# fuxiao0719/PanopticNeRF

Hardware: AMD Instinct MI355X
Metric: Msamples/sec (coarse+fine), KITTI-360 1408x376 (higher is better)
Workload: dtype bf16

## Files before the change

include/pnr.h:

```cpp
#ifndef PNR_H
#define PNR_H
#include <stdint.h>

#ifdef __cplusplus
extern "C" {
#endif

#define PNR_OK 0
#define PNR_EINVAL (-1)
#define PNR_EHIP (-2)
#define PNR_ENODEV (-3)

#define PNR_PREC_BF16 0
#define PNR_PREC_FP32 1

int pnr_version(void);
const char* pnr_last_error(void);
int pnr_device_check(int dev, char* buf_host, int buflen);

int pnr_stratified(const float* rays, int64_t n_rays, int n_samples, int lindisp,
                   const float* t_rand, float* z_out, void* stream);

int pnr_points(const float* rays, const float* z, int64_t n_rays, int n_samples, float* pts_out,
               void* stream);

int pnr_embed(const float* x, int64_t n, int L, float* out, void* stream);

typedef struct pnr_mlp_desc {
    int32_t D, W, skip;
    int32_t xyz_L, dir_L;
    int32_t n_sem, n_inst, head_W;
    int32_t precision;
    int32_t plan;
    int32_t head_tap;
    int32_t head_depth;
    int32_t schedule;
    int32_t clk_probe[2];
    int32_t flags;
} pnr_mlp_desc;

#define PNR_MLP_SOFTMAX 1
#define PNR_MLP_WG_CAP(n) (((n) & 0x1FF) << 16)
#define PNR_MLP_TRACE 0x7A00

typedef struct pnr_mlp_params_host {
    const float* const* pts_w; const float* const* pts_b;
    const float* alpha_w; const float* alpha_b;
    const float* feature_w; const float* feature_b;
    const float* views_w; const float* views_b;
    const float* rgb_w; const float* rgb_b;
    const float* sem0_w; const float* sem0_b; const float* sem1_w; const float* sem1_b;
    const float* inst0_w; const float* inst0_b; const float* inst1_w; const float* inst1_b;
} pnr_mlp_params_host;

int64_t pnr_mlp_packed_bytes(const pnr_mlp_desc* desc);
int pnr_mlp_pack(const pnr_mlp_desc* desc, const pnr_mlp_params_host* params, void* packed_host);

int64_t pnr_mlp_pack_workspace_bytes(const pnr_mlp_desc* desc, int backward);
int pnr_mlp_pack_device(const pnr_mlp_desc* desc, const pnr_mlp_params_host* params_dev, int backward,
                        void* workspace, void* packed, void* stream);
int pnr_mlp_repack_device(const pnr_mlp_desc* desc, const pnr_mlp_params_host* params_dev, int backward,
                          void* workspace, void* packed, void* stream);

int pnr_mlp_forward(const pnr_mlp_desc* desc, const void* packed, const float* rays, const float* z,
                    int64_t n_rays, int n_samples, float* raw, int64_t raw_stride_s,
                    int64_t raw_stride_c, void* stream);

int pnr_mlp_fused_plan(const pnr_mlp_desc* desc);
int64_t pnr_mlp_forward_composite_workspace_bytes(const pnr_mlp_desc* desc, int64_t n_rays, int n_samples, int want_weights);
int pnr_mlp_forward_composite(const pnr_mlp_desc* desc, const void* packed, const float* rays, const float* z,
                              int64_t n_rays, int n_samples, const int32_t* label_sem, const int32_t* label_inst,
                              int white_bkgd, float* rgb, float* depth, float* acc, float* weights, float* sem,
                              float* inst, float* fix_sem, float* fix_inst, void* workspace, void* stream);

int pnr_mlp_forward_tiles(const pnr_mlp_desc* desc, const void* packed, const float* rays, const float* z, int64_t n_rays,
                          int n_samples, void* workspace, void* stream);
int pnr_composite_combine(const pnr_mlp_desc* desc, const void* workspace, const float* z, int64_t n_rays, int n_samples,
                          const int32_t* label_sem, const int32_t* label_inst, int white_bkgd, float* rgb, float* depth,
                          float* acc, float* weights, float* sem, float* inst, float* fix_sem, float* fix_inst, void* stream);

int pnr_mlp_query(const pnr_mlp_desc* desc, const void* packed, const float* points, int64_t n_points,
                  float* sigma, int32_t* sem_label, int32_t* inst_label, int32_t* panoptic, const int32_t* is_thing,
                  float* sem_logits, float* inst_logits, int64_t logit_stride, void* stream);
int pnr_mlp_query_supported(const pnr_mlp_desc* desc);

int pnr_mlp_train_layout(const pnr_mlp_desc* desc, int64_t n_samples, int64_t* acts_off_host ,
                         int64_t* dys_off_host );
int pnr_mlp_forward_train(const pnr_mlp_desc* desc, const void* packed, const float* rays, const float* z,
                          int64_t n_rays, int n_samples, float* raw, int64_t raw_stride_s,
                          int64_t raw_stride_c, void* acts, void* stream);
int64_t pnr_mlp_bwd_packed_bytes(const pnr_mlp_desc* desc);
int pnr_mlp_pack_bwd(const pnr_mlp_desc* desc, const pnr_mlp_params_host* params, void* packed_host);
int pnr_mlp_backward(const pnr_mlp_desc* desc, const void* packed_bwd, const float* d_raw, const void* acts,
                     void* dys, int64_t n_rays, int n_samples, void* stream);

int64_t pnr_mlp_wgrad_workspace_bytes(const pnr_mlp_desc* desc, int64_t n_samples);
int pnr_mlp_wgrad(const pnr_mlp_desc* desc, const void* acts, const void* dys, int64_t n_samples,
                  const pnr_mlp_params_host* grads_dev, void* workspace, void* stream);

int64_t pnr_mlp_fp32_acts_floats(const pnr_mlp_desc* desc, int64_t n_samples);
int64_t pnr_mlp_backward_fp32_workspace_bytes(const pnr_mlp_desc* desc, int64_t n_samples);
int pnr_mlp_forward_train_fp32(const pnr_mlp_desc* desc, const pnr_mlp_params_host* params_dev, const float* rays,
                               const float* z, int64_t n_rays, int n_samples, float* raw, int64_t raw_stride_s,
                               int64_t raw_stride_c, float* acts, void* stream);
int pnr_mlp_backward_fp32(const pnr_mlp_desc* desc, const pnr_mlp_params_host* params_dev, const float* d_raw,
                          int64_t d_raw_stride_c, const float* acts, int64_t n_rays, int n_samples,
                          const pnr_mlp_params_host* grads_dev, void* workspace, void* stream);

int pnr_composite(const float* raw, int64_t raw_stride_s, int64_t raw_stride_c, const float* z,
                  const float* rays, const float* noise, const int32_t* label_sem,
                  const int32_t* label_inst, int64_t n_rays, int n_samples, int n_sem, int n_inst,
                  int sem_mode, int white_bkgd, float* rgb, float* depth, float* acc, float* weights,
                  float* sem, float* inst, float* fix_sem, float* fix_inst, void* stream);

int pnr_composite_backward(const float* raw, int64_t raw_stride_c, const float* z, const float* rays,
                           const float* noise, int64_t n_rays, int n_samples, int n_sem, int n_inst,
                           const float* g_rgb, const float* g_depth, const float* g_acc, const float* g_sem,
                           const float* g_inst, const float* g_weights, float* d_raw, void* stream);

int pnr_composite_backward2(const float* raw, int64_t raw_stride_c, const float* z, const float* rays,
                            const float* noise, int64_t n_rays, int n_samples, int n_sem, int n_inst,
                            const float* g_rgb, const float* g_depth, const float* g_acc, const float* g_sem,
                            const float* g_inst, const float* g_weights, const int32_t* label_sem,
                            const int32_t* label_inst, const float* g_fix_sem, const float* g_fix_inst,
                            const float* ce_sem, const float* ce_inst, float* d_raw, void* stream);
// ... 244 lines not shown
```

panopticnerf_amd/_lib.py:

```python
import ctypes
import os

_HERE = os.path.dirname(os.path.abspath(__file__))
LIB_PATH = os.environ.get("PNR_LIB_PATH") or os.path.join(_HERE, "libpnr.so")

c_f = ctypes.c_void_p
c_i64 = ctypes.c_int64
c_int = ctypes.c_int

PREC_BF16, PREC_FP32 = 0, 1
MLP_SOFTMAX, MLP_TRACE = 1, 0x7A00
CAMERA_PINHOLE, CAMERA_FISHEYE, CAMERA_EQUIRECT = 0, 1, 3
TAG_PIXEL, TAG_FRAME = 16, 17
SAMPLE_POOLED, SAMPLE_FRAME = 0, 1
NORMAL_OK, NORMAL_NO_DEPTH, NORMAL_NO_NEIGHBOUR, NORMAL_DEGENERATE, NORMAL_GRAZING = 0, 1, 2, 3, 4
DEPTH_MAX_RADIUS = 8
NN_MAX_TABLE, CLOUD_MAX_TAU, SAMPLE_MAX_PER_FACE = 1 << 28, 8, 65535


class LossCfg(ctypes.Structure):
    _fields_ = [("w_rgb", ctypes.c_float), ("w_depth", ctypes.c_float), ("w_sem", ctypes.c_float),
                ("w_fix_sem", ctypes.c_float), ("w_inst", ctypes.c_float), ("w_fix_inst", ctypes.c_float),
                ("depth_l2", ctypes.c_int32), ("fix_eps", ctypes.c_float), ("maps_are_prob", ctypes.c_int32)]


class MlpDesc(ctypes.Structure):
    _fields_ = [("D", ctypes.c_int32), ("W", ctypes.c_int32), ("skip", ctypes.c_int32),
                ("xyz_L", ctypes.c_int32), ("dir_L", ctypes.c_int32),
                ("n_sem", ctypes.c_int32), ("n_inst", ctypes.c_int32), ("head_W", ctypes.c_int32),
                ("precision", ctypes.c_int32), ("plan", ctypes.c_int32), ("head_tap", ctypes.c_int32),
                ("head_depth", ctypes.c_int32), ("schedule", ctypes.c_int32), ("clk_probe", ctypes.c_int32 * 2), ("flags", ctypes.c_int32)]


class RngDesc(ctypes.Structure):
    _fields_ = [("call", ctypes.c_void_p), ("ray_base", ctypes.c_int64), ("tag", ctypes.c_int32), ("scale", ctypes.c_float)]


class Frame(ctypes.Structure):
    _fields_ = [("model", ctypes.c_int32), ("width", ctypes.c_int32), ("height", ctypes.c_int32), ("cam", ctypes.c_float * 7),
                ("c2w", ctypes.c_float * 12), ("near_", ctypes.c_float), ("far_", ctypes.c_float), ("n_valid", ctypes.c_int64),
                ("valid_pix", ctypes.c_uint64), ("rgb", ctypes.c_uint64), ("depth", ctypes.c_uint64), ("sem", ctypes.c_uint64),
                ("inst", ctypes.c_uint64)]


_fp = ctypes.POINTER(ctypes.c_float)
_fpp = ctypes.POINTER(_fp)


class MlpParamsHost(ctypes.Structure):
    _fields_ = [("pts_w", _fpp), ("pts_b", _fpp),
                ("alpha_w", _fp), ("alpha_b", _fp), ("feature_w", _fp), ("feature_b", _fp),
                ("views_w", _fp), ("views_b", _fp), ("rgb_w", _fp), ("rgb_b", _fp),
                ("sem0_w", _fp), ("sem0_b", _fp), ("sem1_w", _fp), ("sem1_b", _fp),
                ("inst0_w", _fp), ("inst0_b", _fp), ("inst1_w", _fp), ("inst1_b", _fp)]


SIGNATURES = {
    "pnr_version": (c_int, []),
    "pnr_last_error": (ctypes.c_char_p, []),
    "pnr_device_check": (c_int, [c_int, ctypes.c_char_p, c_int]),
    "pnr_stratified": (c_int, [c_f, c_i64, c_int, c_int, c_f, c_f, c_f]),
    "pnr_points": (c_int, [c_f, c_f, c_i64, c_int, c_f, c_f]),
    "pnr_embed": (c_int, [c_f, c_i64, c_int, c_f, c_f]),
    "pnr_mlp_packed_bytes": (c_i64, [ctypes.POINTER(MlpDesc)]),
    "pnr_mlp_pack": (c_int, [ctypes.POINTER(MlpDesc), ctypes.POINTER(MlpParamsHost), ctypes.c_void_p]),
    "pnr_mlp_pack_workspace_bytes": (c_i64, [ctypes.POINTER(MlpDesc), c_int]),
    "pnr_mlp_pack_device": (c_int, [ctypes.POINTER(MlpDesc), ctypes.POINTER(MlpParamsHost), c_int, c_f, c_f, c_f]),
    "pnr_mlp_repack_device": (c_int, [ctypes.POINTER(MlpDesc), ctypes.POINTER(MlpParamsHost), c_int, c_f, c_f, c_f]),
    "pnr_mlp_forward": (c_int, [ctypes.POINTER(MlpDesc), c_f, c_f, c_f, c_i64, c_int, c_f, c_i64, c_i64, c_f]),
    "pnr_mlp_train_layout": (c_int, [ctypes.POINTER(MlpDesc), c_i64, ctypes.POINTER(c_i64), ctypes.POINTER(c_i64)]),
    "pnr_mlp_forward_train": (c_int, [ctypes.POINTER(MlpDesc), c_f, c_f, c_f, c_i64, c_int, c_f, c_i64, c_i64, c_f, c_f]),
    "pnr_mlp_bwd_packed_bytes": (c_i64, [ctypes.POINTER(MlpDesc)]),
    "pnr_mlp_pack_bwd": (c_int, [ctypes.POINTER(MlpDesc), ctypes.POINTER(MlpParamsHost), ctypes.c_void_p]),
    "pnr_mlp_backward": (c_int, [ctypes.POINTER(MlpDesc), c_f, c_f, c_f, c_f, c_i64, c_int, c_f]),
    "pnr_mlp_wgrad_workspace_bytes": (c_i64, [ctypes.POINTER(MlpDesc), c_i64]),
    "pnr_mlp_wgrad": (c_int, [ctypes.POINTER(MlpDesc), c_f, c_f, c_i64, ctypes.POINTER(MlpParamsHost), c_f, c_f]),
    "pnr_mlp_fp32_acts_floats": (c_i64, [ctypes.POINTER(MlpDesc), c_i64]),
    "pnr_mlp_backward_fp32_workspace_bytes": (c_i64, [ctypes.POINTER(MlpDesc), c_i64]),
    "pnr_mlp_forward_train_fp32": (c_int, [ctypes.POINTER(MlpDesc), ctypes.POINTER(MlpParamsHost), c_f, c_f, c_i64, c_int, c_f, c_i64,
                                           c_i64, c_f, c_f]),
    "pnr_mlp_backward_fp32": (c_int, [ctypes.POINTER(MlpDesc), ctypes.POINTER(MlpParamsHost), c_f, c_i64, c_f, c_i64, c_int,
                                      ctypes.POINTER(MlpParamsHost), c_f, c_f]),
    "pnr_mlp_fused_plan": (c_int, [ctypes.POINTER(MlpDesc)]),
    "pnr_mlp_forward_composite_workspace_bytes": (c_i64, [ctypes.POINTER(MlpDesc), c_i64, c_int, c_int]),
    "pnr_mlp_forward_composite": (c_int, [ctypes.POINTER(MlpDesc), c_f, c_f, c_f, c_i64, c_int, c_f, c_f, c_int,
                                          c_f, c_f, c_f, c_f, c_f, c_f, c_f, c_f, c_f, c_f]),
    "pnr_composite": (c_int, [c_f, c_i64, c_i64, c_f, c_f, c_f, c_f, c_f, c_i64, c_int, c_int, c_int, c_int,
                              c_int, c_f, c_f, c_f, c_f, c_f, c_f, c_f, c_f, c_f]),
    "pnr_composite_backward": (c_int, [c_f, c_i64, c_f, c_f, c_f, c_i64, c_int, c_int, c_int,
                                       c_f, c_f, c_f, c_f, c_f, c_f, c_f, c_f]),
    "pnr_composite_backward2": (c_int, [c_f, c_i64, c_f, c_f, c_f, c_i64, c_int, c_int, c_int,
                                        c_f, c_f, c_f, c_f, c_f, c_f, c_f, c_f, c_f, c_f, c_f, c_f, c_f, c_f]),
    "pnr_composite_backward3": (c_int, [c_f, c_i64, c_f, c_f, c_f, c_i64, c_int, c_int, c_int, c_int,
                                        c_f, c_f, c_f, c_f, c_f, c_f, c_f, c_f, c_f, c_f, c_f, c_f, c_f, c_f]),
# ... 105 lines not shown
```

panopticnerf_amd/csrc/asm/gen_mlp_tt.py:

```python
#!/usr/bin/env python3
import struct
import sys
from contextlib import contextmanager

V_T2 = 15
NSLOT, SLOT = 4, 33 * 1024
P = 4
D, SKIP = 8, 4

V_TID, V_LANE16, V_FRAG, V_BIAS, V_T0, V_DMA, V_LB4, V_TRACE = 0, 1, 2, 6, 10, 11, 14, 15
V_T1 = 1
V_RING, V_ACC = 16, 32
V_EX, V_ED = 160, 192
V_G = 208
V_ZZ, V_ZN, V_DN, V_LW = 240, 242, 244, 246
V_IN = 224
V_TMP = 208
V_PTMP = 248
V_AUXA = V_PTMP + 6
V_LWA = V_IN + 2
A0, A1 = 0, 128
S_IMG, S_RAYS, S_Z, S_S, S_N, S_MAGIC, S_SHIFT, S_NGRP, S_NWG, S_REC, S_RECF, S_PS, S_NSEM, S_NINST, S_CLK = 4, 6, 8, 10, 11, 12, 13, 14, 15, 16, 18, 20, 22, 23, 24
S_WAVE, S_W4K, S_GRP, S_PIECE, S_T0, S_T1 = 26, 27, 28, 30, 34, 35
S_VALID, S_LAST = 36, 40
S_NVALID, S_NLAST = 44, 48
S_LO32, S_N0, S_HI0 = 52, 54, 56
S_SAVE, S_REC_T = 58, 60
S_MSK = 64
S_REC_I = 70
S_AUX = 82
S_VMSK = 76
S_LWW, S_LWR = 74, 75
LW_BASE = NSLOT * SLOT
S_CLK0 = 96
S_K = 100
S_Q = 19
S_GRP2 = 29


def f32(x):
    return struct.unpack("<I", struct.pack("<f", x))[0]


def vr(lo, n):
    return "v[%d:%d]" % (lo, lo + n - 1) if n > 1 else "v%d" % lo


def ar(lo, n):
    return "a[%d:%d]" % (lo, lo + n - 1) if n > 1 else "a%d" % lo


def sr(lo, n=2):
    return "s[%d:%d]" % (lo, lo + n - 1) if n > 1 else "s%d" % lo


class Loc:
    def __init__(self, kind, base):
        self.kind, self.base = kind, base

    def reg(self, i, n=1):
        return (ar if self.kind == "a" else vr)(self.base + i, n)


class Sim:
    def __init__(self, name, cap):
        self.name, self.cap, self.q, self.n = name, cap, [], 0

    def push(self, certain=True):
        self.n += 1
        self.q.append((self.n, certain))
        return self.n

    def wait_count(self, tag):
        if tag is None or not any(t == tag for t, _ in self.q):
            return None
        idx = [t for t, _ in self.q].index(tag)
        n = sum(1 for _, c in self.q[idx + 1:] if c)
        n = min(n, self.cap)
        self.q = self.q[idx + 1:]
        return n

    def drain(self):
        self.q = []

    def state(self):
        return [c for _, c in self.q]


class Gen:
    def __init__(self, nbs, nbi, name, trace=False, abl=0, depth=2, softmax=False, tap=0):
        self.depth = depth
        self.tap = tap
        self.softmax = softmax
        self.nbs, self.nbi, self.name, self.trace, self.abl = nbs, nbi, name, trace, abl
        self.nstamp = 0
        self.o = []
        self.nlabel = 0
        self.lgkm = Sim("lgkm", 15)
        self.vm = Sim("vm", 63)
        self.side, self.side_lo, self.outbox, self.capture = [], [], [], None
        self.ring_tags = [None] * P
        self.piece_tag = {}
        self.pending_pack = None
        self.g2_acc = self.park_acc = None
        self.m0 = None
        self.logit_units = []
        self.acc_free = list(range(8))
        self.lwr_acc = self.lwr_tag = None
        self.aux_tags = {}
        self.build_plan()
        self.build_units()
        self.stream = []
        for u in self.units:
            u["frag0"] = len(self.stream)
            self.stream += [(sl, of) for sl, of, _, _ in self.unit_frags(u)]

    def build_plan(self):
        L = []

        def add(name, nblk, segs, fbc, mode):
            nks = sum(n for _, n in segs)
            if fbc * nks + 1 > 33:
                fbc = 1
            L.append(dict(name=name, nblk=nblk, segs=segs, nks=nks, fbc=fbc, mode=mode))
        for i in range(D):
            if i == 0:
                add("L0", 8, [("ex", 4)], 8, "relu")
            elif i - 1 == SKIP:
                add("L%d" % i, 8, [("ex", 4), ("h", 16)], 2, "relu")
            else:
                add("L%d" % i, 8, [("h", 16)], 2, "relu")
        add("feature", 8, [("h", 16)], 2, "linear")
        add("views", 4, [("F", 16), ("ed", 2)], 2, "relu")
        add("rgbs", 1, [("g", 8), ("hh", 16)], 1, "rgbs")
        if self.depth == 1:
            if self.nbs:
                add("sem1", self.nbs, [("tap", 16)], self.nbs, "logits")
            if self.nbi:
                add("inst1", 1, [("tap", 16)], 1, "logits")
        else:
            if self.nbs:
                add("sem0", 4, [("tap", 16)], 2, "relu")
            if self.nbi:
                add("inst0", 4, [("tap", 16)], 2, "relu")
            if self.nbs:
                add("sem1", self.nbs, [("shs", 8)], self.nbs, "logits")
            if self.nbi:
                add("inst1", 1, [("shi", 8)], 1, "logits")
        self.layers = L
        self.chunks = []
        off = 0
        for li, l in enumerate(L):
            for fb in range(0, l["nblk"], l["fbc"]):
                nfrag = l["fbc"] * l["nks"] + 1
                self.chunks.append(dict(layer=li, fb=fb, nfb=l["fbc"], off=off, nfrag=nfrag))
                off += nfrag
        self.total_frags = off
        while len(self.chunks) % NSLOT:
            self.chunks.append(dict(layer=None, fb=0, nfb=0, off=0, nfrag=1, dummy=True))
        self.NC = len(self.chunks)
        assert self.NC % NSLOT == 0, self.NC
        assert max(c["nfrag"] for c in self.chunks) <= 33

    class Holder:
        def __init__(self, v=None):
            self.v = v

    def e(self, s):
        if self.capture is not None:
            self.capture.append("\t" + s)
        else:
            self.o.append("\t" + s)

# ... 229 lines not shown
        e("v_fma_f32 v%d, -v%d, v%d, v%d" % (a, a, q_, b))
        e("v_div_fmas_f32 v%d, v%d, v%d, v%d" % (a, a, r, q_))
        e("v_div_fixup_f32 v%d, v%d, v%d, v%d" % (res, a, den, num))

    def sqrt(self, res, x, t):
        y, ym, tt = t[:3]
        e = self.e
        self.lit(S_K, 0x0f800000)
        e("v_mul_f32 v%d, 0x4f800000, v%d" % (tt, x))
        e("v_cmp_gt_f32 vcc, s%d, v%d" % (S_K, x))
        e("v_cndmask_b32 v%d, v%d, v%d, vcc" % (x, x, tt))
        e("v_sqrt_f32 v%d, v%d" % (y, x))
        e("s_nop 0")
        e("v_add_u32 v%d, -1, v%d" % (ym, y))
        e("v_fma_f32 v%d, -v%d, v%d, v%d" % (tt, ym, y, x))
        e("v_cmp_ge_f32 s[%d:%d], 0, v%d" % (S_T0, S_T0 + 1, tt))
        e("v_cndmask_b32 v%d, v%d, v%d, s[%d:%d]" % (ym, y, ym, S_T0, S_T0 + 1))
        e("v_add_u32 v%d, 1, v%d" % (tt, y))
        e("v_fma_f32 v%d, -v%d, v%d, v%d" % (y, tt, y, x))
        e("v_cmp_lt_f32 s[%d:%d], 0, v%d" % (S_T0, S_T0 + 1, y))
        e("v_cndmask_b32 v%d, v%d, v%d, s[%d:%d]" % (ym, ym, tt, S_T0, S_T0 + 1))
        e("v_mul_f32 v%d, 0x37800000, v%d" % (tt, ym))
        e("v_cndmask_b32 v%d, v%d, v%d, vcc" % (ym, ym, tt))
        e("v_mov_b32 v%d, 0x260" % tt)
        e("v_cmp_class_f32 vcc, v%d, v%d" % (x, tt))
        e("v_cndmask_b32 v%d, v%d, v%d, vcc" % (res, ym, x))

    def sincos(self, s_out, c_out, x, t):
        kf, r, r2, a, b, ki = t[:6]
        e = self.e
        C = dict(twoopi=f32(0.636619772367581343), c1=f32(1.57079637050628662109375), c2=f32(-4.371139000186241e-08),
                 s3=f32(-1.9515295891e-4), s2=f32(8.3321608736e-3), s1=f32(-1.6666654611e-1),
                 c4=f32(2.443315711809948e-5), c3=f32(-1.388731625493765e-3), c2b=f32(4.166664568298827e-2))
        assert C["twoopi"] == 0x3f22f983 and C["c1"] == 0x3fc90fdb and C["c2"] == 0xb33bbd2e and C["s3"] == 0xb94ca1f9
        assert C["s2"] == 0x3c08839e and C["s1"] == 0xbe2aaaa3 and C["c4"] == 0x37ccf5ce and C["c3"] == 0xbab6061a and C["c2b"] == 0x3d2aaaa5
        e("v_mul_f32 v%d, 0x%x, v%d" % (kf, C["twoopi"], x))
        e("v_rndne_f32 v%d, v%d" % (kf, kf))
        e("v_mov_b32 v%d, v%d" % (r, x))
        e("v_fmac_f32 v%d, 0x%x, v%d" % (r, C["c1"] ^ 0x80000000, kf))
        e("v_fmac_f32 v%d, 0x%x, v%d" % (r, C["c2"] ^ 0x80000000, kf))
        e("v_cvt_i32_f32 v%d, v%d" % (ki, kf))
        e("v_mul_f32 v%d, v%d, v%d" % (r2, r, r))
        e("v_mov_b32 v%d, 0x%x" % (a, C["s2"]))
        e("v_fmac_f32 v%d, 0x%x, v%d" % (a, C["s3"], r2))
        e("v_fmaak_f32 v%d, v%d, v%d, 0x%x" % (a, r2, a, C["s1"]))
        e("v_mul_f32 v%d, v%d, v%d" % (b, r, r2))
        e("v_fma_f32 v%d, v%d, v%d, v%d" % (a, b, a, r))
        e("v_mov_b32 v%d, 0x%x" % (b, C["c3"]))
        e("v_fmac_f32 v%d, 0x%x, v%d" % (b, C["c4"], r2))
        e("v_fmaak_f32 v%d, v%d, v%d, 0x%x" % (b, r2, b, C["c2b"]))
        e("v_fma_f32 v%d, v%d, v%d, -0.5" % (b, r2, b))
        e("v_fma_f32 v%d, v%d, v%d, 1.0" % (b, r2, b))
        e("v_and_b32 v%d, 1, v%d" % (r, ki))
        e("v_cmp_eq_u32 vcc, 0, v%d" % r)
        e("v_cndmask_b32 v%d, v%d, v%d, vcc" % (r2, b, a))
        e("v_cndmask_b32 v%d, v%d, v%d, vcc" % (kf, a, b))
        e("v_and_b32 v%d, 2, v%d" % (a, ki))
        e("v_lshlrev_b32 v%d, 30, v%d" % (a, a))
        e("v_xor_b32 v%d, v%d, v%d" % (s_out, r2, a))
        e("v_add_u32 v%d, 1, v%d" % (a, ki))
        e("v_and_b32 v%d, 2, v%d" % (a, a))
        e("v_lshlrev_b32 v%d, 30, v%d" % (a, a))
        e("v_xor_b32 v%d, v%d, v%d" % (c_out, kf, a))

    def band_pack(self, dst3, s, c):
        e = self.e
        e("v_cvt_pk_bf16_f32 v%d, v%d, v%d" % (dst3, s[0], s[1]))
        e("v_cvt_pk_bf16_f32 v%d, v%d, v%d" % (dst3 + 1, s[2], c[0]))
        e("v_cvt_pk_bf16_f32 v%d, v%d, v%d" % (dst3 + 2, c[1], c[2]))

    def band_next(self, s, c, t):
        e = self.e
        for a in range(3):
            e("v_add_f32 v%d, v%d, v%d" % (t, s[a], s[a]))
            e("v_mul_f32 v%d, v%d, v%d" % (t, t, c[a]))
            e("v_mul_f32 v%d, -2.0, v%d" % (c[a], s[a]))
            e("v_fma_f32 v%d, v%d, v%d, 1.0" % (c[a], c[a], s[a]))
            e("v_mov_b32 v%d, v%d" % (s[a], t))

    def fetch_tile(self, t, grp_sreg):
        e = self.e
        vi = V_IN + 8 * t
        s_, sl, ray, a64 = V_PTMP, V_PTMP + 1, V_PTMP + 2, V_PTMP + 4
        e("s_lshl_b32 s%d, s%d, 3" % (S_T0, grp_sreg))
        e("s_lshl_b32 s%d, s%d, 1" % (S_T1, S_WAVE))
        e("s_add_u32 s%d, s%d, s%d" % (S_T0, S_T0, S_T1))
        e("s_add_u32 s%d, s%d, %d" % (S_T0, S_T0, t))
        e("s_lshl_b32 s%d, s%d, 5" % (S_T0, S_T0))
        e("v_and_b32 v%d, 31, v%d" % (s_, V_TID))
        e("v_or_b32 v%d, s%d, v%d" % (s_, S_T0, s_))
        e("v_cmp_gt_i32 s[%d:%d], s%d, v%d" % (S_NVALID + 2 * t, S_NVALID + 2 * t + 1, S_S, s_))
        e("s_add_i32 s%d, s%d, -1" % (S_T1, S_S))
        e("v_min_i32 v%d, s%d, v%d" % (sl, S_T1, s_))
        e("v_mul_hi_u32 v%d, v%d, s%d" % (ray, sl, S_MAGIC))
        e("v_mul_lo_u32 v%d, v%d, s%d" % (a64, sl, S_MAGIC))
        e("v_mov_b32 v%d, v%d" % (a64 + 1, ray))
        e("v_lshrrev_b64 v[%d:%d], s%d, v[%d:%d]" % (a64, a64 + 1, S_SHIFT, a64, a64 + 1))
        e("v_mov_b32 v%d, v%d" % (ray, a64))
        e("v_mul_lo_u32 v%d, v%d, s%d" % (a64, ray, S_N))
        e("v_sub_u32 v%d, v%d, v%d" % (a64, sl, a64))
        e("v_add_u32 v%d, 1, v%d" % (a64, a64))
        e("v_cmp_eq_u32 s[%d:%d], s%d, v%d" % (S_NLAST + 2 * t, S_NLAST + 2 * t + 1, S_N, a64))
        e("v_lshlrev_b32 v%d, 7, v%d" % (V_AUXA + t, ray))
        e("v_and_b32 v%d, 32, v%d" % (a64, V_TID))
        e("v_lshl_add_u32 v%d, v%d, 1, v%d" % (V_AUXA + t, a64, V_AUXA + t))
        e("v_lshlrev_b32 v%d, 5, v%d" % (a64, ray))
        self.vm_op("global_load_dwordx4 %s, v%d, s[%d:%d]" % (vr(vi, 4), a64, S_RAYS, S_RAYS + 1))
        self.vm_op("global_load_dwordx2 %s, v%d, s[%d:%d] offset:16" % (vr(vi + 4, 2), a64, S_RAYS, S_RAYS + 1))
        e("v_lshlrev_b32 v%d, 2, v%d" % (a64, sl))
        self.vm_op("global_load_dword v%d, v%d, s[%d:%d]" % (vi + 6, a64, S_Z, S_Z + 1))
        e("v_add_u32 v%d, 1, v%d" % (a64 + 1, sl))
        e("v_cmp_gt_i32 vcc, s%d, v%d" % (S_S, a64 + 1))
        e("v_cndmask_b32 v%d, v%d, v%d, vcc" % (a64 + 1, sl, a64 + 1))
        e("v_lshlrev_b32 v%d, 2, v%d" % (a64 + 1, a64 + 1))
        return self.vm_op("global_load_dword v%d, v%d, s[%d:%d]" % (vi + 7, a64 + 1, S_Z, S_Z + 1))

    def encode_tile(self, t, part):
        vi = V_IN + 8 * t
        T = list(range(V_TMP, V_TMP + 16))
        s = T[0:3]
        c = T[3:6]
        q = T[6:9]
        w = T[9:15]
        tt = T[15]
        e = self.e
        ex, ed = V_EX + 16 * t, V_ED + 8 * t
        out = []

        def hi_select(dst, v_hi1, v_hi0):
            e("v_cndmask_b32 v%d, v%d, v%d, s[%d:%d]" % (dst, v_hi1, v_hi0, S_HI0, S_HI0 + 1))

        def points():
            for a in range(3):
                e("v_mul_f32 v%d, v%d, v%d" % (q[a], vi + 3 + a, vi + 6))
                e("v_add_f32 v%d, v%d, v%d" % (q[a], vi + a, q[a]))
        if part == "x":
            out.append((6, points))

        def aux_x():
            self.aux_tags[t] = self.vm_op("global_load_dword v%d, v%d, s[%d:%d] offset:32" % (vi + 0, V_AUXA + t, S_AUX, S_AUX + 1))
            e("v_mov_b32 v%d, v%d" % (vi + 3, V_AUXA + t))
        if part == "x":
            out.append((2, aux_x))

        def xyz_reg():
            hi_select(w[0], q[2], q[0])
            e("v_mov_b32 v%d, 0" % w[1])
            hi_select(w[1], w[1], q[1])
            e("v_cvt_pk_bf16_f32 v%d, v%d, v%d" % (ex, w[0], w[1]))
            e("v_mov_b32 v%d, 0x42000000" % tt)
            e("v_mov_b32 v%d, 1.0" % w[1])
            hi_select(tt, tt, w[1])
            for a in range(3):
                e("v_mul_f32 v%d, v%d, v%d" % (q[a], q[a], tt))
        if part == "x":
            out.append((12, xyz_reg))
            for a in range(3):
                out.append((30, (lambda a=a: self.sincos(s[a], c[a], q[a], w))))
            for fp in range(5):
                out.append((3, (lambda fp=fp: self.band_pack(ex + 1 + 3 * fp, s, c))))
                if fp < 4:
                    out.append((15, (lambda: self.band_next(s, c, tt))))

        if part == "x":
            out.append((1, (lambda: self.wait_vm(self.aux_tags[t]))))
            return out

        def d_load():
            self.vm_op("global_load_dwordx4 %s, v%d, s[%d:%d]" % (vr(ed, 4), vi + 3, S_AUX, S_AUX + 1))
            self.aux_tags[2 + t] = self.vm_op("global_load_dwordx4 %s, v%d, s[%d:%d] offset:16" % (vr(ed + 4, 4), vi + 3, S_AUX, S_AUX + 1))
        out.append((2, d_load))
        out.append((1, (lambda: self.wait_vm(self.aux_tags[2 + t]))))
        return out

    def rgbs_epilogue(self, t, acc):
        e = self.e
        T = list(range(V_PTMP, V_PTMP + 8))
        d, x, y, n, al, f = T[0], T[1], T[2], T[3], T[4], T[5]
        VAL, LAST = S_VALID + 2 * t, S_LAST + 2 * t

        def alpha():
            e("v_sub_f32 v%d, v%d, v%d" % (d, V_ZN + t, V_ZZ + t))
            e("v_mov_b32 v%d, 0x501502f9" % x)
            e("v_cndmask_b32 v%d, v%d, v%d, s[%d:%d]" % (d, d, x, LAST, LAST + 1))
            e("v_mul_f32 v%d, v%d, -v%d" % (d, d, V_DN + t))
            e("v_max_f32 v%d, v%d, v%d" % (x, acc + 3, acc + 3))
            e("v_max_f32 v%d, 0, v%d" % (x, x))
            e("v_mul_f32 v%d, v%d, v%d" % (x, d, x))
            self.lit(S_K, 0x3fb8aa3b)
            e("v_mul_f32 v%d, 0x3fb8aa3b, v%d" % (y, x))
            e("v_fma_f32 v%d, v%d, s%d, -v%d" % (d, x, S_K, y))
            e("v_rndne_f32 v%d, v%d" % (n, y))
            e("v_fmac_f32 v%d, 0x32a5705f, v%d" % (d, x))
            e("v_sub_f32 v%d, v%d, v%d" % (y, y, n))
            e("v_add_f32 v%d, v%d, v%d" % (y, y, d))
            e("v_exp_f32 v%d, v%d" % (y, y))
            e("v_cvt_i32_f32 v%d, v%d" % (n, n))
            e("s_nop 0")
            e("v_ldexp_f32 v%d, v%d, v%d" % (y, y, n))
            self.lit(S_K, 0xc2ce8ed0)
            e("v_cmp_ngt_f32 s[%d:%d], s%d, v%d" % (S_T0, S_T0 + 1, S_K, x))
            e("v_cndmask_b32 v%d, 0, v%d, s[%d:%d]" % (y, y, S_T0, S_T0 + 1))
            self.lit(S_K, 0x42b17218)
            e("v_cmp_nlt_f32 s[%d:%d], s%d, v%d" % (S_T0, S_T0 + 1, S_K, x))
            e("v_mov_b32 v%d, 0x7f800000" % n)
            e("v_cndmask_b32 v%d, v%d, v%d, s[%d:%d]" % (y, n, y, S_T0, S_T0 + 1))
            e("v_sub_f32 v%d, 1.0, v%d" % (al, y))
            e("v_cndmask_b32 v%d, 0, v%d, s[%d:%d]" % (al, al, VAL, VAL + 1))
            e("v_sub_f32 v%d, 1.0, v%d" % (f, al))
            e("v_add_f32 v%d, 0x2edbe6ff, v%d" % (f, f))
            e("v_mov_b32 v%d, 1.0" % n)
            e("v_cndmask_b32 v%d, v%d, v%d, s[%d:%d]" % (f, n, f, VAL, VAL + 1))
        self.q(36, alpha)

        def scan():
            for ctrl in ("row_shr:1", "row_shr:2", "row_shr:4", "row_shr:8"):
                e("v_mov_b32 v%d, 1.0" % n)
                e("s_nop 1")
                e("v_mov_b32_dpp v%d, v%d %s row_mask:0xf bank_mask:0xf" % (n, f, ctrl))
                e("v_mul_f32 v%d, v%d, v%d" % (f, f, n))
            e("v_mov_b32 v%d, 1.0" % n)
            e("s_nop 1")
            e("v_mov_b32_dpp v%d, v%d row_bcast:15 row_mask:0xa bank_mask:0xf" % (n, f))
            e("v_mul_f32 v%d, v%d, v%d" % (f, f, n))
            e("v_mov_b32 v%d, 1.0" % n)
            e("s_nop 1")
            e("v_readlane_b32 s%d, v%d, 31" % (S_Q, f))
            e("v_mov_b32_dpp v%d, v%d wave_shr:1 row_mask:0xf bank_mask:0xf" % (n, f))
            e("v_cndmask_b32 v%d, v%d, 1.0, s[%d:%d]" % (n, n, S_N0, S_N0 + 1))
            e("v_mul_f32 v%d, v%d, v%d" % (V_LW + t, al, n))
            if self.nbs:
                with self.atomic():
                    e("v_add_u32 v%d, s%d, v%d" % (n, S_LWW, V_LB4))
                    e("s_mov_b64 exec, s[%d:%d]" % (S_HI0, S_HI0 + 1))
                    self.lds_read("ds_write_b32 v%d, v%d offset:%d" % (n, V_LW + t, 128 * t))
                    e("s_mov_b64 exec, -1")
        self.q(26 + (4 if self.nbs else 0), scan)

        def stores():
          with self.atomic():
            e("s_lshl_b32 s%d, s%d, 3" % (S_T0, S_GRP))
            e("s_lshl_b32 s%d, s%d, 1" % (S_SAVE, S_WAVE))
            e("s_add_u32 s%d, s%d, s%d" % (S_T0, S_T0, S_SAVE))
            e("s_add_u32 s%d, s%d, %d" % (S_T0, S_T0, t))
            e("s_mul_i32 s%d, s%d, s%d" % (S_SAVE, S_T0, S_RECF))
            e("s_mul_hi_i32 s%d, s%d, s%d" % (S_SAVE + 1, S_T0, S_RECF))
            e("s_lshl_b64 s[%d:%d], s[%d:%d], 2" % (S_SAVE, S_SAVE + 1, S_SAVE, S_SAVE + 1))
            e("s_add_u32 s%d, s%d, s%d" % (S_REC_T + 2 * t, S_REC, S_SAVE))
            e("s_addc_u32 s%d, s%d, s%d" % (S_REC_T + 2 * t + 1, S_REC + 1, S_SAVE + 1))
            e("s_lshl_b32 s%d, s%d, 2" % (S_SAVE, S_NSEM))
            e("s_add_u32 s%d, s%d, s%d" % (S_REC_I + 2 * t, S_REC_T + 2 * t, S_SAVE))
            e("s_addc_u32 s%d, s%d, 0" % (S_REC_I + 2 * t + 1, S_REC_T + 2 * t + 1))
            e("s_lshl_b32 s%d, s%d, 5" % (S_T0, S_T0))
            e("v_and_b32 v%d, 31, v%d" % (d, V_TID))
            e("v_or_b32 v%d, s%d, v%d" % (d, S_T0, d))
            e("v_lshlrev_b32 v%d, 4, v%d" % (d, d))
            e("v_mov_b32 v%d, v%d" % (T[4], V_LW + t))
            e("v_mov_b32 v%d, v%d" % (T[5], acc + 0))
            e("v_mov_b32 v%d, v%d" % (T[6], acc + 1))
            e("v_mov_b32 v%d, v%d" % (T[7], acc + 2))
            e("s_and_b64 s[%d:%d], s[%d:%d], s[%d:%d]" % (S_SAVE, S_SAVE + 1, VAL, VAL + 1, S_HI0, S_HI0 + 1))
            e("s_mov_b64 exec, s[%d:%d]" % (S_SAVE, S_SAVE + 1))
            self.vm_op("global_store_dwordx4 v%d, %s, s[%d:%d]" % (d, vr(T[4], 4), S_PS, S_PS + 1))
            e("s_mov_b64 exec, 1")
            e("v_mov_b32 v%d, s%d" % (x, S_Q))
            e("v_mov_b32 v%d, 0" % d)
            self.vm_op("global_store_dword v%d, v%d, s[%d:%d]" % (d, x, S_REC_T + 2 * t, S_REC_T + 2 * t + 1))
            e("s_mov_b64 exec, -1")
        self.q(28, stores)

    def acc_reg(self, i):
        return V_ACC + 16 * i

    def acc_take(self, n):
        assert len(self.acc_free) >= n, ("accumulators exhausted", self.acc_free)
        got, self.acc_free = self.acc_free[:n], self.acc_free[n:]
        return got

    def acc_release(self, ids):
        self.acc_free = sorted(set(self.acc_free) | set(ids))

    def arm_plan(self, u):
        c = self.chunks[u["chunk"]]
        l = self.layers[u["layer"]]
        slot = u["chunk"] % NSLOT
        bias_off = c["nfb"] * l["nks"] * 1024
        u["accs"], u["arm_tags"] = {}, []
        plans = []
        for bi, blk in enumerate(u["blocks"]):
            b_in_chunk = blk - c["fb"]
            for t in range(2):
                key = (bi, t)
                ops = []

                def take(key=key):
                    while not self.acc_free and self.side_busy():
                        self.drain_side(8)
                    u["accs"][key] = self.acc_take(1)[0]
                if t == 1:
                    plans.append([take])
                    continue
                if l["mode"] == "logits":
                    def first(key=key, slot=slot, take=take):
                        take()
                        self.e("v_add_u32 v%d, 0x%x, v%d" % (self.acc_reg(u["accs"][key]), slot * SLOT, V_LB4))
                    ops.append(first)
                    for r in list(range(1, 16)) + [0]:
                        ops.append(lambda key=key, r=r, off=bias_off + b_in_chunk * 128: u["arm_tags"].append(
                            self.lds_read("ds_read_b32 v%d, v%d offset:%d" % (self.acc_reg(u["accs"][key]) + r, self.acc_reg(u["accs"][key]), off))))
                else:
                    for m in range(4):
                        def rd(key=key, m=m, off=bias_off + b_in_chunk * 128 + m * 32, take=take):
                            if m == 0:
                                take()
                            a = self.acc_reg(u["accs"][key])
                            u["arm_tags"].append(self.lds_read("ds_read_b128 %s, v%d offset:%d" % (vr(a + 4 * m, 4), V_BIAS + slot, off)))
                        ops.append(rd)
                plans.append(ops)
        return plans

    def pack_ops(self, u):
        l = self.layers[u["layer"]]
        if not self.trace:
            return self.pack_ops_pipelined(u)
        out = []
        for bi, blk in enumerate(u["blocks"]):
            for t in range(2):
                a = self.acc_reg(u["accs"][(bi, t)])
                dst = self.out_block(l, blk, t)
                for p in range(8):
                    def fn(a=a, p=p, dst=dst, relu=(l["mode"] == "relu"), k=len(out)):
                        tmp = V_T0 if (k & 1) else V_T1
                        if dst.kind == "v" and relu:
                            self.e("v_cvt_pk_bf16_f32 v%d, v%d, v%d" % (tmp, a + 2 * p, a + 2 * p + 1))
                            self.e("v_pk_max_i16 v%d, v%d, 0" % (dst.base + p, tmp))
                        elif dst.kind == "v":
                            self.e("v_cvt_pk_bf16_f32 v%d, v%d, v%d" % (dst.base + p, a + 2 * p, a + 2 * p + 1))
                        else:
                            self.e("v_cvt_pk_bf16_f32 v%d, v%d, v%d" % (tmp, a + 2 * p, a + 2 * p + 1))
                            if relu:
                                self.e("v_pk_max_i16 v%d, v%d, 0" % (tmp, tmp))
                            self.e("v_accvgpr_write_b32 a%d, v%d" % (dst.base + p, tmp))
                    out.append(((dst.kind, dst.base + p), fn, u["accs"][(bi, t)]))
        return out

    def pack_ops_pipelined(self, u):
        l = self.layers[u["layer"]]
        relu = l["mode"] == "relu"
        pairs = []
        for bi, blk in enumerate(u["blocks"]):
            for t in range(2):
                a = self.acc_reg(u["accs"][(bi, t)])
# ... 97 lines not shown
                    dls.append(None)
                k += 1
        for kk in range(k, len(plans)):
            for op in plans[kk]:
                musts.append(op)
                dls.append(None)
        lwr_from = None
        if nxt is None and (self.logit_units or l["mode"] == "logits"):
            lwr_from = len(musts)
            for op in self.lwr_ops():
                musts.append(op)
                dls.append(None)
        n = len(musts)
        pos = []
        late = not packs and n > 0 and nxt is not None
        for j in range(n):
            spread = 1 + (j * max(1, nm - 6)) // max(1, n) if not late else (2 * nm) // 3 + (j * max(1, nm // 3 - 5)) // max(1, n)
            pos.append(spread if dls[j] is None else min(spread, max(0, dls[j] - 2)))
        if lwr_from is not None:
            nl = n - lwr_from
            for j in range(lwr_from, n):
                pos[j] = max(pos[j], min(nm - 2, nm // 2 + ((j - lwr_from) * max(1, nm // 2 - 3)) // nl))
        for j in range(n - 2, -1, -1):
            pos[j] = min(pos[j], pos[j + 1])
        must_at = {}
        for j, g in enumerate(pos):
            must_at.setdefault(g, []).append(j)
        piece_at = {}
        cu = [k for k, x in enumerate(U) if x["chunk"] == u["chunk"]]
        c3 = (u["chunk"] + 3) % self.NC
        npieces = self.pieces_of(c3)
        k_in = cu.index(ui)
        mine = [j for j in range(npieces) if (j * len(cu)) // npieces == k_in]
        cost = [3 * sum(1 for j in must_at.get(g, []) if j < n and dls[j] is not None or (j < n and musts[j] in pack_fns)) +
                sum(1 for j in must_at.get(g, [])) for g in range(nm)]
        for idx, j in enumerate(mine):
            span = max(len(mine) + 1, nm - 3)
            lo = 1 + (idx * span) // max(1, len(mine))
            hi = max(lo + 1, 1 + ((idx + 1) * span) // max(1, len(mine)))
            g = min(range(lo, min(hi, nm - 1)), key=lambda x: (cost[x], x))
            cost[g] += 2
            piece_at.setdefault(g, []).append(j)
        first_wait_done = False
        for i in range(nm):
            f, t = i // 2, i % 2
            slot, off, ks, bi = frags[f]
            gi = u["frag0"] + f
            if t == 0:
                if not first_wait_done:
                    for tg in u["arm_tags"][-1:]:
                        self.wait_lgkm(tg)
                    first_wait_done = True
                self.wait_lgkm(self.ring_tags[gi % P])
            tile = self.tile_at(ks, t)
            a = self.acc_reg(u["accs"][(bi, tile)])
            c_in = self.acc_reg(u["accs"][(bi, 0)]) if ks == 0 else a
            bloc = self.b_operand(u, ks, tile)
            ring = vr(V_RING + 4 * (gi % P), 4)
            if swap:
                e("v_mfma_f32_32x32x16_bf16 %s, %s, %s, %s" % (vr(a, 16), bloc.reg(0, 4), ring, vr(c_in, 16)))
            else:
                e("v_mfma_f32_32x32x16_bf16 %s, %s, %s, %s" % (vr(a, 16), ring, bloc.reg(0, 4), vr(c_in, 16)))
            if t == 1:
                gn = gi + P - 1
                if gn < len(self.stream):
                    sl, of = self.stream[gn]
                    self.ring_tags[gn % P] = self.lds_read("ds_read_b128 %s, v%d offset:%d" % (vr(V_RING + 4 * (gn % P), 4), V_FRAG + sl, of))
            for j in must_at.get(i, []):
                musts[j]()
            for j in ([] if self.abl & 1 else piece_at.get(i, [])):
                if j == 0:
                    self.chunk_base(c3)
                tg = self.piece(c3, j)
                self.piece_tag[c3] = tg
            self.drain_side(1 if l["name"].startswith("L") or l["name"] in ("feature", "views") else 3 if late else 2)
        for g in sorted(must_at):
            assert g < nm, (g, nm)
        if l["mode"] in ("relu", "linear"):
            self.pending_pack = dict(ops=self.pack_ops(u), accs=list(u["accs"].values()))
        elif l["mode"] == "rgbs":
            for t in range(2):
                self.rgbs_epilogue(t, self.acc_reg(u["accs"][(0, t)]))
            ids = list(u["accs"].values())
            self.q(0, lambda: self.defer(lambda: self.acc_release(ids)))
            self.queue_inputs_late()
            self.acc_release([self.g2_acc])
            self.g2_acc = None
            if not self.nbs:
                self.unpark()
        else:
            self.logit_units.append(u)
        if u["last_of_chunk"]:
            c2 = (u["chunk"] + 2) % self.NC
            if not self.abl & 2:
                self.wait_vm(self.piece_tag.get(c2))
                e("s_barrier")
            d = u["chunk"] + 1
            while d < self.NC and self.chunks[d].get("dummy"):
                e("; ==== dummy chunk %d (slot %d)" % (d, d % NSLOT))
                c3 = (d + 3) % self.NC
                for j in ([] if self.abl & 1 else range(self.pieces_of(c3))):
                    if j == 0:
                        self.chunk_base(c3)
                    self.piece_tag[c3] = self.piece(c3, j)
                    self.drain_side(2)
                if not self.abl & 2:
                    self.wait_vm(self.piece_tag.get((d + 2) % self.NC))
                    e("s_barrier")
                d += 1

    def tail_softmax(self, blocks, lwr_reg, tag_lwr):
        e = self.e
        M = (V_TMP, V_RING)
        TMP = [V_IN + 10, V_IN + 11, V_IN + 12, V_IN + 13]
        ninf = V_PTMP + 6
        heads = []
        for inst in (False, True):
            hb = [(u, bi, blk) for (u, bi, blk, i2) in blocks if i2 == inst]
            if hb:
                heads.append((inst, hb))
        for t in (0, 1):
            self.wait_lgkm(tag_lwr[t])
        e("v_mov_b32 v%d, 0xff800000" % ninf)

        def xor16(op):
            regs = [M[t] + r for t in (0, 1) for r in range(16)]
            for g in range(0, 32, 4):
                for i in range(4):
                    e("v_mov_b32 v%d, v%d" % (TMP[i], regs[g + i]))
                for i in range(4):
                    e("v_permlane16_swap_b32 v%d, v%d" % (regs[g + i], TMP[i]))
                for i in range(4):
                    e("%s v%d, v%d, v%d" % (op, regs[g + i], regs[g + i], TMP[i]))
        for inst, hb in heads:
            accs = [[self.acc_reg(u["accs"][(bi, t)]) for (u, bi, blk) in hb] for t in (0, 1)]
            NB = len(hb)
            vm = S_VMSK + 2 * (1 if inst else 0)
            for t in (0, 1):
                for r in range(16):
                    e("v_cndmask_b32 v%d, v%d, v%d, s[%d:%d]" % (accs[t][NB - 1] + r, ninf, accs[t][NB - 1] + r, vm, vm + 1))
            first_src = None
            if NB > 1:
                for t in (0, 1):
                    for r in range(16):
                        e("v_max_f32 v%d, v%d, v%d" % (M[t] + r, accs[t][0] + r, accs[t][1] + r))
                        for b in range(2, NB):
                            e("v_max_f32 v%d, v%d, v%d" % (M[t] + r, M[t] + r, accs[t][b] + r))
            else:
                first_src = [accs[t][0] for t in (0, 1)]
            for k, ctrl in enumerate(("quad_perm:[1,0,3,2]", "quad_perm:[2,3,0,1]", "row_half_mirror", "row_mirror")):
                for t in (0, 1):
                    for r in range(16):
                        src = (first_src[t] + r) if (k == 0 and first_src) else (M[t] + r)
                        e("v_max_f32_dpp v%d, v%d, v%d %s row_mask:0xf bank_mask:0xf bound_ctrl:1" % (M[t] + r, src, src, ctrl))
            xor16("v_max_f32")
            for t in (0, 1):
                for r in range(16):
                    e("v_mul_f32 v%d, 0xbfb8aa3b, v%d" % (M[t] + r, M[t] + r))
            for t in (0, 1):
                for r in range(16):
                    for b in range(NB):
                        e("v_fmamk_f32 v%d, v%d, 0x3fb8aa3b, v%d" % (accs[t][b] + r, accs[t][b] + r, M[t] + r))
                        e("v_exp_f32 v%d, v%d" % (accs[t][b] + r, accs[t][b] + r))
            first_src = None
            if NB > 1:
                for t in (0, 1):
                    for r in range(16):
# ... 15 lines not shown
                for r in range(16):
                    e("v_mul_f32 v%d, v%d, v%d" % (M[t] + r, lwr_reg(t, r), M[t] + r))
            for r in range(16):
                for t in (0, 1):
                    for (u, bi, blk) in hb:
                        kk = [i for i, (u2, bi2, blk2, i2) in enumerate(blocks) if u2 is u and bi2 == bi][0]
                        a = self.acc_reg(u["accs"][(bi, t)])
                        dst = self.sm_sums[t][kk]
                        if r == 0:
                            e("v_fma_f32 v%d, v%d, v%d, 0" % (dst, M[t], a))
                        else:
                            e("v_fmac_f32 v%d, v%d, v%d" % (dst, M[t] + r, a + r))

    def lwr_ops(self):
        ops = []

        def first():
            while self.side or self.outbox or (len(self.acc_free) < 2 and self.side_busy()):
                self.drain_side(8)
            assert len(self.acc_free) >= 2, ("no free accumulators for the local weights", self.acc_free)
            self.lwr_acc = self.acc_take(2)
            self.e("v_add_u32 v%d, s%d, v%d" % (V_LWA, S_LWR, V_BIAS + 0))
        ops.append(first)
        for t in range(2):
            for q in range(4):
                for h2 in range(2):
                    def rd(t=t, q=q, h2=h2):
                        dst = self.acc_reg(self.lwr_acc[t]) + 4 * q + ((2 * h2 + 2) & 3)
                        self.lwr_tag = self.lds_read("ds_read_b64 %s, v%d offset:%d" % (vr(dst, 2), V_LWA, 128 * t + 32 * q + 8 * h2))
                    ops.append(rd)
        return ops

    def logit_blocks(self):
        return [(b, False) for b in range(self.nbs)] + [(0, True)] * self.nbi

    def tail_logits(self):
        e = self.e
        if not self.logit_units:
            return
        blocks = []
        for u in self.logit_units:
            inst = self.layers[u["layer"]]["name"] == "inst1"
            for bi, blk in enumerate(u["blocks"]):
                blocks.append((u, bi, blk, inst))
        nb = len(blocks)
        lwr = tuple(self.acc_reg(a) for a in self.lwr_acc)

        def lwr_reg(t, r):
            return lwr[t] + 4 * (r >> 2) + (((r & 3) + 2) & 3)
        sums = ([V_PTMP + k for k in range(nb)], [V_IN + 1 + k for k in range(nb)])
        oth = ([V_PTMP + 3 + k for k in range(nb)], [V_IN + 4, V_IN + 5, V_IN + 9][:nb])
        adr = V_PTMP + 7
        tag_lwr = [self.lwr_tag, self.lwr_tag]
        e("v_xor_b32 v%d, 32, v%d" % (adr, V_TID))
        e("v_and_b32 v%d, 63, v%d" % (adr, adr))
        e("v_lshlrev_b32 v%d, 2, v%d" % (adr, adr))
        tags = [None, None]

        self.sm_sums = sums

        def fmas(ts):
            for t in ts:
                self.wait_lgkm(tag_lwr[t])
            for r in ([] if self.softmax else range(16)):
                for t in ts:
                    for k, (u, bi, blk, inst) in enumerate(blocks):
                        a = self.acc_reg(u["accs"][(bi, t)])
                        if r == 0:
                            e("v_fma_f32 v%d, v%d, v%d, 0" % (sums[t][k], lwr_reg(t, 0), a))
                        else:
                            e("v_fmac_f32 v%d, v%d, v%d" % (sums[t][k], lwr_reg(t, r), a + r))
            for t in ts:
                tags[t] = [self.lds_read("ds_bpermute_b32 v%d, v%d, v%d" % (oth[t][k], adr, sums[t][k])) for k in range(nb)]

        def stores(t):
            for k in range(nb):
                self.wait_lgkm(tags[t][k])
                e("v_add_f32 v%d, v%d, v%d" % (oth[t][k], sums[t][k], oth[t][k]))
            for k, (u, bi, blk, inst) in enumerate(blocks):
                e("s_mov_b64 exec, s[%d:%d]" % (S_MSK + 2 * k, S_MSK + 2 * k + 1))
                base = (S_REC_I if inst else S_REC_T) + 2 * t
                self.vm_op("global_store_dword v%d, v%d, s[%d:%d] offset:%d" % (V_LB4, oth[t][k], base, base + 1, 4 + 128 * blk))
            e("s_mov_b64 exec, -1")
        self.stamp(len(self.units) + 4)
        if self.softmax:
            self.tail_softmax(blocks, lwr_reg, tag_lwr)
        fmas((0, 1))
        self.stamp(len(self.units) + 5)
        stores(0)
        stores(1)
        for u in self.logit_units:
            self.acc_release(list(u["accs"].values()))
        self.acc_release(self.lwr_acc)
        self.lwr_acc = None
        self.logit_units = []

    def queue_inputs_early(self):
        def which():
            with self.atomic():
                self.e("s_add_u32 s%d, s%d, s%d" % (S_GRP2, S_GRP, S_NWG))
                self.e("s_cmp_lt_i32 s%d, s%d" % (S_GRP2, S_NGRP))
                self.e("s_cselect_b32 s%d, s%d, s%d" % (S_GRP2, S_GRP2, S_GRP))
        self.q(3, which)
        tags = {}
        for t in range(2):
            self.q(34, (lambda t=t: tags.__setitem__(t, self.fetch_tile(t, S_GRP2))))
        for t in range(2):
            self.q(1, (lambda t=t: self.wait_vm(tags[t])))
            for cost, fn in self.encode_tile(t, "x"):
                self.q(cost, fn)

    PARK = (3, 6, 7, 0)

    def park(self):
        self.park_acc = self.acc_take(1)[0]
        for t in range(2):
            for i, k in enumerate(Gen.PARK):
                self.e("v_mov_b32 v%d, v%d" % (self.acc_reg(self.park_acc) + len(Gen.PARK) * t + i, V_IN + 8 * t + k))

    def unpark(self):
        for t in range(2):
            for i, k in enumerate(Gen.PARK):
                self.e("v_mov_b32 v%d, v%d" % (V_IN + 8 * t + k, self.acc_reg(self.park_acc) + len(Gen.PARK) * t + i))
        self.acc_release([self.park_acc])
        self.park_acc = None

    def queue_inputs_late(self):
        for t in range(2):
            for cost, fn in self.encode_tile(t, "d"):
                self.q(cost, fn, low=True)

    def stamp(self, idx):
        if not self.trace:
            return
        pair = S_CLK0 + 2 * (self.nstamp & 1)
        prev = S_CLK0 + 2 * ((self.nstamp + 1) & 1)
        if self.last_stamp is not None:
            self.o.append("\tv_writelane_b32 v%d, s%d, %d" % (V_TRACE, prev, self.last_stamp))
        self.o.append("\ts_memtime s[%d:%d]" % (pair, pair + 1))
        self.last_stamp = idx
        self.nstamp += 1
        if idx == len(self.units) + 3:
            skip = self.label()
            self.o += ["\ts_waitcnt lgkmcnt(0)", "\ts_and_b32 s%d, s101, 7" % S_T0, "\ts_add_u32 s%d, s%d, 56" % (S_T0, S_T0),
                       "\ts_mov_b32 m0, s%d" % S_T0, "\ts_nop 1",
                       "\tv_writelane_b32 v%d, s%d, m0" % (V_TRACE, pair),
                       "\ts_and_b32 s%d, s101, 31" % S_T0, "\ts_cmp_eq_u32 s%d, 0" % S_T0, "\ts_cbranch_scc0 %s" % skip,
                       "\ts_lshr_b32 s%d, s101, 5" % S_T0, "\ts_add_u32 s%d, s%d, 48" % (S_T0, S_T0), "\ts_mov_b32 m0, s%d" % S_T0,
                       "\ts_nop 1", "\tv_writelane_b32 v%d, s%d, m0" % (V_TRACE, pair), skip + ":",
                       "\ts_add_u32 s101, s101, 1"]

    def prefetch_first_unit(self):
        u0 = self.units[0]
        for plan in self.arm_plan(u0):
            for op in plan:
                op()
        for g in range(P - 1):
            sl, of = self.stream[g]
            self.ring_tags[g % P] = self.lds_read("ds_read_b128 %s, v%d offset:%d" % (vr(V_RING + 4 * (g % P), 4), V_FRAG + sl, of))

    def advance_group_state(self):
        e = self.e
        for t in range(2):
            vi = V_IN + 8 * t
            e("v_mov_b32 v%d, v%d" % (V_ZZ + t, vi + 6))
            e("v_mov_b32 v%d, v%d" % (V_ZN + t, vi + 7))
            e("v_mov_b32 v%d, v%d" % (V_DN + t, vi + 0))
            e("s_mov_b64 s[%d:%d], s[%d:%d]" % (S_VALID + 2 * t, S_VALID + 2 * t + 1, S_NVALID + 2 * t, S_NVALID + 2 * t + 1))
            e("s_mov_b64 s[%d:%d], s[%d:%d]" % (S_LAST + 2 * t, S_LAST + 2 * t + 1, S_NLAST + 2 * t, S_NLAST + 2 * t + 1))

    def group_body(self):
        self.m0 = None
        assert self.acc_free == [i for i in range(8) if i not in self.units[0]["accs"].values()], self.acc_free
        self.last_stamp = None
        for ui in range(len(self.units)):
            self.emit_unit(ui)
        self.stamp(len(self.units))
        self.drain_side()
        self.tail_logits()
        self.stamp(len(self.units) + 1)
        assert self.acc_free == list(range(8)), self.acc_free
        self.e("s_waitcnt lgkmcnt(0)")
        self.lgkm.drain()
        self.advance_group_state()
        self.stamp(len(self.units) + 2)
        if self.trace:
            self.o.append("\ts_waitcnt lgkmcnt(0)")
            self.stamp(len(self.units) + 3)

    def kernel(self):
        e, name = self.e, self.name
        self.o += ["\t.text", "\t.globl\t%s" % name, "\t.p2align\t8", "\t.type\t%s,@function" % name, "%s:" % name]
        for dst, off, n in ((S_IMG, 0x0, 2), (S_RAYS, 0x8, 2), (S_Z, 0x10, 2), (S_S, 0x18, 2), (S_MAGIC, 0x20, 2), (S_NGRP, 0x28, 2),
                            (S_REC, 0x30, 2), (S_RECF, 0x38, 1), (S_PS, 0x40, 2), (S_NSEM, 0x48, 2), (S_CLK, 0x50, 2), (S_AUX, 0x58, 2)):
            e("s_load_dword%s %s, s[0:1], 0x%x" % ("x2" if n == 2 else "", sr(dst, n), off))
        e("v_readfirstlane_b32 s%d, v0" % S_WAVE)
        e("s_nop 4")
        e("s_lshr_b32 s%d, s%d, 6" % (S_WAVE, S_WAVE))
        e("s_lshl_b32 s%d, s%d, 12" % (S_W4K, S_WAVE))
        e("v_and_b32 v%d, 63, v0" % V_T0)
        e("v_lshlrev_b32 v%d, 4, v%d" % (V_LANE16, V_T0))
        e("v_lshrrev_b32 v%d, 5, v0" % V_LB4)
        e("v_and_b32 v%d, 1, v%d" % (V_LB4, V_LB4))
        e("v_lshlrev_b32 v%d, 4, v%d" % (V_LB4, V_LB4))
        for sl in range(NSLOT):
            self.lit(S_T0, sl * SLOT)
            e("v_add_u32 v%d, s%d, v%d" % (V_FRAG + sl, S_T0, V_LANE16))
            e("v_add_u32 v%d, s%d, v%d" % (V_BIAS + sl, S_T0, V_LB4))
        for k in range(3):
            e("v_add_u32 v%d, s%d, v%d" % (V_DMA + k, S_W4K, V_LANE16))
            if k:
                e("v_add_u32 v%d, 0x%x, v%d" % (V_DMA + k, 16384 * k, V_DMA + k))
        e("v_and_b32 v%d, 31, v0" % V_LB4)
        e("v_lshlrev_b32 v%d, 2, v%d" % (V_LB4, V_LB4))
        e("s_mov_b32 s%d, -1" % S_LO32)
        e("s_mov_b32 s%d, 0" % (S_LO32 + 1))
        e("s_mov_b32 s%d, 1" % S_N0)
        e("s_mov_b32 s%d, 1" % (S_N0 + 1))
        e("s_mov_b32 s%d, -1" % S_HI0)
        e("s_mov_b32 s%d, 0" % (S_HI0 + 1))
        e("s_lshr_b32 s%d, s%d, 4" % (S_LWW, S_W4K))
        e("s_add_u32 s%d, s%d, 0x%x" % (S_LWW, S_LWW, LW_BASE))
        e("s_sub_u32 s%d, s%d, 0x%x" % (S_LWR, S_LWW, 0 * SLOT))
        e("s_waitcnt lgkmcnt(0)")
        for k, (blk, inst) in enumerate(self.logit_blocks()):
            e("v_and_b32 v%d, 31, v0" % V_T0)
            if blk:
                e("v_add_u32 v%d, %d, v%d" % (V_T0, 32 * blk, V_T0))
            e("v_cmp_gt_i32 vcc, s%d, v%d" % (S_NINST if inst else S_NSEM, V_T0))
            e("s_and_b64 s[%d:%d], vcc, s[%d:%d]" % (S_MSK + 2 * k, S_MSK + 2 * k + 1, S_HI0, S_HI0 + 1))
        if self.softmax:
            for k, (nblk, sreg) in enumerate(((self.nbs, S_NSEM), (self.nbi, S_NINST))):
                if nblk:
                    e("v_and_b32 v%d, 31, v0" % V_T0)
                    if nblk > 1:
                        e("v_add_u32 v%d, %d, v%d" % (V_T0, 32 * (nblk - 1), V_T0))
                    e("v_cmp_gt_i32 s[%d:%d], s%d, v%d" % (S_VMSK + 2 * k, S_VMSK + 2 * k + 1, sreg, V_T0))
        lend, lloop, lfin = self.label(), self.label(), self.label()
        e("s_mov_b32 s%d, s2" % S_GRP)
        e("s_cmp_ge_i32 s%d, s%d" % (S_GRP, S_NGRP))
        e("s_cbranch_scc1 %s" % lend)
        for c in range(3):
            self.chunk_base(c)
            for j in range(self.pieces_of(c)):
                self.piece_tag[c] = self.piece(c, j)
        e("s_waitcnt vmcnt(0)")
        self.vm.drain()
        e("s_barrier")
        e("s_mov_b32 s%d, s%d" % (S_GRP2, S_GRP))
        tags = [self.fetch_tile(t, S_GRP2) for t in range(2)]
        for t in range(2):
            self.wait_vm(tags[t])
            for part in ("x", "d"):
                for _, fn in self.encode_tile(t, part):
                    fn()
        self.advance_group_state()
        if not self.trace:
            e("s_memtime s[%d:%d]" % (S_CLK0, S_CLK0 + 1))
            e("s_memrealtime s[%d:%d]" % (S_CLK0 + 2, S_CLK0 + 3))
        else:
            e("v_mov_b32 v%d, 0" % V_TRACE)
            e("s_mov_b32 s101, 0")
            e("s_memtime s[90:91]")
            e("s_waitcnt lgkmcnt(0)")
        e("s_waitcnt lgkmcnt(0)")
        self.lgkm.drain()
        self.prefetch_first_unit()
        keep = self.o
        self.o = []
        self.group_body()
        self.prefetch_first_unit()
        self.o = keep
        self.o.append(lloop + ":")
        self.group_body()
        e("s_add_u32 s%d, s%d, s%d" % (S_GRP, S_GRP, S_NWG))
        e("s_cmp_ge_i32 s%d, s%d" % (S_GRP, S_NGRP))
        e("s_cbranch_scc1 %s" % lend)
        self.prefetch_first_unit()
        e("s_branch %s" % lloop)
        self.o.append(lend + ":")
        e("s_waitcnt vmcnt(0) lgkmcnt(0)")
        e("s_cmp_eq_u64 s[%d:%d], 0" % (S_CLK, S_CLK + 1))
        e("s_cbranch_scc1 %s" % lfin)
        if self.trace:
            lw = self.label()
            e("s_cmp_lg_u32 s%d, 0" % S_WAVE)
            e("s_cbranch_scc1 %s" % lw)
            e("s_memtime s[%d:%d]" % (S_CLK0, S_CLK0 + 1))
            e("s_waitcnt lgkmcnt(0)")
            e("s_sub_u32 s%d, s%d, s90" % (S_CLK0, S_CLK0))
            e("s_lshl_b32 s%d, s2, 2" % S_T0)
            e("s_add_u32 s%d, s%d, 256" % (S_T0, S_T0))
            e("v_mov_b32 v%d, s%d" % (V_T0, S_T0))
            e("v_mov_b32 v%d, s%d" % (V_T1, S_CLK0))
            e("s_mov_b64 exec, 1")
            e("global_store_dword v%d, v%d, s[%d:%d]" % (V_T0, V_T1, S_CLK, S_CLK + 1))
            e("s_mov_b64 exec, -1")
            e("s_waitcnt vmcnt(0)")
            self.o.append(lw + ":")
        e("s_cmp_lg_u32 s2, 0")
        e("s_cbranch_scc1 %s" % lfin)
        if self.trace:
            e("s_cmp_lg_u32 s%d, 0" % S_WAVE)
            e("s_cbranch_scc1 %s" % lfin)
            e("v_and_b32 v%d, 63, v0" % V_T0)
            e("v_lshlrev_b32 v%d, 2, v%d" % (V_T0, V_T0))
            e("global_store_dword v%d, v%d, s[%d:%d]" % (V_T0, V_TRACE, S_CLK, S_CLK + 1))
            e("s_waitcnt vmcnt(0)")
            e("s_branch %s" % lfin)
        e("s_memtime s[%d:%d]" % (S_T0 - 0, S_T0 + 1))
        e("s_memrealtime s[%d:%d]" % (S_SAVE, S_SAVE + 1))
        e("s_waitcnt lgkmcnt(0)")
        e("s_sub_u32 s%d, s%d, s%d" % (S_T0, S_T0, S_CLK0))
        e("s_subb_u32 s%d, s%d, s%d" % (S_T1, S_T1, S_CLK0 + 1))
        e("s_sub_u32 s%d, s%d, s%d" % (S_SAVE, S_SAVE, S_CLK0 + 2))
        e("s_subb_u32 s%d, s%d, s%d" % (S_SAVE + 1, S_SAVE + 1, S_CLK0 + 3))
        e("v_cmp_eq_u32 vcc, 0, v0")
        e("s_and_saveexec_b64 s[%d:%d], vcc" % (S_VALID, S_VALID + 1))
        e("s_cbranch_execz %s" % lfin)
        e("v_mov_b32 v20, s%d" % S_T0)
        e("v_mov_b32 v21, s%d" % S_T1)
        e("v_mov_b32 v22, s%d" % S_SAVE)
        e("v_mov_b32 v23, s%d" % (S_SAVE + 1))
        e("v_mov_b32 v%d, 0" % V_T0)
        e("global_store_dwordx4 v%d, v[20:23], s[%d:%d]" % (V_T0, S_CLK, S_CLK + 1))
        e("s_waitcnt vmcnt(0)")
        self.o.append(lfin + ":")
        e("s_endpgm")
        self.o += [".Lend_%s:" % name, "\t.size\t%s, .Lend_%s-%s" % (name, name, name), ""]
        self.o += ["\t.rodata", "\t.p2align\t6", "\t.amdhsa_kernel %s" % name,
                   "\t\t.amdhsa_group_segment_fixed_size %d" % (NSLOT * SLOT + 1024),
                   "\t\t.amdhsa_private_segment_fixed_size 0", "\t\t.amdhsa_kernarg_size %d" % KERNARG_BYTES, "\t\t.amdhsa_user_sgpr_count 2",
                   "\t\t.amdhsa_user_sgpr_kernarg_segment_ptr 1", "\t\t.amdhsa_system_sgpr_workgroup_id_x 1",
                   "\t\t.amdhsa_system_vgpr_workitem_id 0", "\t\t.amdhsa_next_free_vgpr 512", "\t\t.amdhsa_next_free_sgpr 102",
                   "\t\t.amdhsa_accum_offset 256", "\t\t.amdhsa_reserve_vcc 1", "\t\t.amdhsa_float_denorm_mode_32 3",
                   "\t\t.amdhsa_float_denorm_mode_16_64 3", "\t\t.amdhsa_dx10_clamp 1", "\t\t.amdhsa_ieee_mode 1",
                   "\t.end_amdhsa_kernel", ""]
        return "\n".join(self.o)


KERNARG_BYTES = 104


def metadata(names):
    o = ["\t.amdgpu_metadata", "---", "amdhsa.kernels:"]
    for n in names:
        o += ["  - .agpr_count:     256", "    .args:", "      - .offset:         0", "        .size:           %d" % KERNARG_BYTES,
              "        .value_kind:     by_value", "    .group_segment_fixed_size: %d" % (NSLOT * SLOT + 1024),
              "    .kernarg_segment_align: 8", "    .kernarg_segment_size: %d" % KERNARG_BYTES, "    .max_flat_workgroup_size: 256",
              "    .name:           %s" % n, "    .private_segment_fixed_size: 0", "    .sgpr_count:     108",
              "    .sgpr_spill_count: 0", "    .symbol:         %s.kd" % n, "    .uniform_work_group_size: 1",
              "    .uses_dynamic_stack: false", "    .vgpr_count:     512", "    .vgpr_spill_count: 0", "    .wavefront_size: 64"]
    o += ["amdhsa.target:   amdgcn-amd-amdhsa--gfx950", "amdhsa.version:", "  - 1", "  - 2", "...", "\t.end_amdgpu_metadata", ""]
    return "\n".join(o)


def variant_name(tap, depth, sm, nbs, nbi):
    tag = ("f" if tap else "") + ("d1" if depth == 1 else "") + ("sm" if sm else "")
    return "k_mlp_tt_%ss%di%d" % (tag + "_" if tag else "", nbs, nbi)


def main():
    out = sys.argv[1] if len(sys.argv) > 1 else "/dev/stdout"
    parts = ['\t.amdgcn_target "amdgcn-amd-amdhsa--gfx950"', "\t.amdhsa_code_object_version 5", ""]
    names = []
    for nbs, nbi in ((1, 1), (2, 1), (0, 0), (1, 0), (2, 0), (3, 0)):
        n = "k_mlp_tt_s%di%d" % (nbs, nbi)
        names.append(n)
        parts.append(Gen(nbs, nbi, n).kernel())
    for tap in (0, 1):
        for depth in (2, 1):
            for sm in (False, True):
                if (tap, depth, sm) == (0, 2, False):
                    continue
                for nbs, nbi in ((1, 1), (2, 1), (1, 0), (2, 0), (3, 0)):
                    n = variant_name(tap, depth, sm, nbs, nbi)
                    names.append(n)
                    parts.append(Gen(nbs, nbi, n, depth=depth, softmax=sm, tap=tap).kernel())
    extra = sys.argv[3] if len(sys.argv) > 3 else ""
    if extra in ("trace", "abl"):
        names.append("k_mlp_tt_s2i1_trace")
        parts.append(Gen(2, 1, "k_mlp_tt_s2i1_trace", trace=True).kernel())
    if extra == "abl":
        for abl in (1, 2, 3, 4, 7):
            names.append("k_mlp_tt_s2i1_trace_a%d" % abl)
            parts.append(Gen(2, 1, names[-1], trace=True, abl=abl).kernel())
    unit_names = ["%s %s" % (g.layers[u["layer"]]["name"], u["blocks"]) for g in [Gen(2, 1, "x")] for u in g.units]
    if len(sys.argv) > 2:
        open(sys.argv[2], "w").write("\n".join(unit_names) + "\n")
    parts.append(metadata(names))
    with open(out, "w") as f:
        f.write("\n".join(parts))


if __name__ == "__main__":
    main()
```

panopticnerf_amd/csrc/pnr_mlp.hip:

```cpp
#include <stdlib.h>
#include <string.h>

#include "pnr_mlp_plan.h"

int pnr_mlp_validate(const pnr_mlp_desc* d);

#include "pnr_mlp_core.h"
#include "pnr_mlp_pp.h"
#include "pnr_mlp_fuse.h"
#include "pnr_mlp_tt.h"
#define PNR_QUERY_MAX_POINTS (((int64_t)1 << 31) - 4096)
template <int PREC, int TILES, class CTX, int KIND, int NA, int NB, int NFB_OUT, int MODE, int NOUT>
__device__ __forceinline__ void layer_regs(CTX& c, const uint32_t (&inA)[TILES][NA],
                                           const uint32_t (&inB)[TILES][NB > 0 ? NB : 1],
                                           uint32_t (&out)[TILES][NOUT], uint16_t* save = nullptr,
                                           const int* srow = nullptr)
{
    constexpr int RPB = PrecT<PREC>::RPB;
    constexpr int KS = NA / 4 + NB / 4;
    constexpr int FBC0 = pnr_layer_fbc(KIND, PREC);
    constexpr int FBC = (NFB_OUT % FBC0 == 0) ? FBC0 : 1;
    constexpr int G = (CTX::GDB / FBC) < 1 ? 1 : (CTX::GDB / FBC);
    static_assert(NOUT >= NFB_OUT * RPB, "output register array too small");
#pragma unroll
// ... 730 lines not shown
static int mlp_forward_impl(const pnr_mlp_desc* desc, const void* packed, const float* rays, const float* z,
                            int64_t n_rays, int n_samples, float* raw, int64_t raw_stride_s, int64_t raw_stride_c,
                            void* acts, void* stream)
{
    int rc = pnr_mlp_validate(desc);
    if (rc != PNR_OK) return rc;
    PNR_REQUIRE(n_rays >= 0 && n_samples >= 1, "pnr_mlp_forward: bad size");
    if (n_rays == 0) return PNR_OK;
    PNR_REQUIRE(packed && rays && z && raw, "pnr_mlp_forward: null pointer");
    PNR_REQUIRE(n_rays * (int64_t)n_samples < ((int64_t)1 << 31) - 4096, "pnr_mlp_forward: R*N=%lld exceeds 2^31",
                (long long)(n_rays * n_samples));
    PNR_REQUIRE((((uintptr_t)rays) & 15) == 0 && (((uintptr_t)packed) & 15) == 0 && (((uintptr_t)acts) & 15) == 0,
                "pnr_mlp_forward: rays / packed / acts must be 16-byte aligned");
    PNR_REQUIRE(!acts || desc->precision == PNR_PREC_BF16, "pnr_mlp_forward_train: the training path is bf16 only");
    PNR_REQUIRE(desc->plan != 4, "pnr_mlp_forward: a plan-4 (field) image is for pnr_mlp_query only");
    PNR_REQUIRE(desc->plan == 0, "pnr_mlp_forward: plan=%d images are for pnr_mlp_forward_composite only", desc->plan);
    PnrPlan plan;
    pnr_build_plan(*desc, plan);
    MlpArgs a;
    mlp_args_fill(a, desc, plan, packed);
    a.rays = rays; a.z = z; a.S = (int)(n_rays * n_samples); a.N = n_samples;
    pnr_set_div_magic(n_samples, a.n_magic, a.n_shift);
    a.raw = raw; a.ss = raw_stride_s; a.sc = raw_stride_c;
    a.acts = (uint16_t*)acts;
    if (acts) pnr_train_layout(*desc, a.S, a.acts_off, a.dys_off, a.gate_off);
    hipStream_t st = (hipStream_t)stream;
    if (desc->precision == PNR_PREC_BF16) {
        if (desc->schedule != 1 && !acts)
            return desc->W == 256 ? launch_mlp_pp<256, false>(a, st) : launch_mlp_pp<128, false>(a, st);
        if (desc->schedule == 2 && acts)
            return desc->W == 256 ? launch_mlp_pp<256, true>(a, st) : launch_mlp_pp<128, true>(a, st);
        if (acts)
            return desc->W == 256 ? launch_mlp<PNR_PREC_BF16, 256, 1, 8, 2, true>(a, st)
                                  : launch_mlp<PNR_PREC_BF16, 128, 1, 8, 2, true>(a, st);
        return desc->W == 256 ? launch_mlp<PNR_PREC_BF16, 256, 1, 8, 2>(a, st) : launch_mlp<PNR_PREC_BF16, 128, 1, 8, 2>(a, st);
    }
    return desc->W == 256 ? launch_mlp<PNR_PREC_FP32, 256, 1, 4, 1>(a, st) : launch_mlp<PNR_PREC_FP32, 128, 1, 4, 1>(a, st);
}

PNR_EXPORT int pnr_mlp_forward(const pnr_mlp_desc* desc, const void* packed, const float* rays, const float* z,
                               int64_t n_rays, int n_samples, float* raw, int64_t raw_stride_s,
                               int64_t raw_stride_c, void* stream)
{
    return mlp_forward_impl(desc, packed, rays, z, n_rays, n_samples, raw, raw_stride_s, raw_stride_c, nullptr, stream);
}

#define PNR_RAY_AUX_BYTES 128
int pnr_composite_combine_launch(const float* rec, int rec_floats, bool logit_sums, const float4* ps, const float* z,
                                 const int32_t* label_sem, const int32_t* label_inst, int64_t R, int N, int C, int K, int white_bkgd,
                                 float* rgb, float* depth, float* acc, float* weights, float* sem, float* inst, float* fix_sem,
                                 float* fix_inst, hipStream_t st);

static int record_floats(const pnr_mlp_desc& d)
{
    return d.plan == 3 ? pnr_fuse_record_floats(0, 0) : pnr_fuse_record_floats(d.n_sem, d.n_inst);
}

PNR_EXPORT int64_t pnr_mlp_forward_composite_workspace_bytes(const pnr_mlp_desc* desc, int64_t n_rays, int n_samples, int want_weights)
{
    (void)want_weights;
    if (pnr_mlp_validate(desc) != PNR_OK || n_rays < 0 || n_samples < 32 || (n_samples & 31)) return -1;
    const int64_t S = n_rays * n_samples, tiles = (S + 255) / 256 * 8;
    if (desc->plan == 3) return tiles * record_floats(*desc) * 4 + S * 16 + 256;
    return tiles * pnr_fuse_record_floats(desc->n_sem, desc->n_inst) * 4 + S * 16 + 256 + PNR_RAY_AUX_BYTES + n_rays * PNR_RAY_AUX_BYTES;
}

__global__ void __launch_bounds__(256) k_ray_aux(const float* __restrict__ rays, int64_t R, uint32_t* __restrict__ aux)
{
    const int64_t i = (int64_t)blockIdx.x * 256 + threadIdx.x;
    if (i >= 2 * R) return;
    const int64_t ray = i >> 1;
    const int hi = (int)(i & 1);
    const float dx = rays[ray * 8 + 3], dy = rays[ray * 8 + 4], dz = rays[ray * 8 + 5];
    const float nrm = sqrtf(__fadd_rn(__fadd_rn(__fmul_rn(dx, dx), __fmul_rn(dy, dy)), __fmul_rn(dz, dz)));
    uint32_t ed[8];
    embed_lane<PNR_PREC_BF16, 2, 16, 8>(dx / nrm, dy / nrm, dz / nrm, hi, ed);
    uint4* o = reinterpret_cast<uint4*>(aux + i * 16);
    o[0] = make_uint4(ed[0], ed[1], ed[2], ed[3]);
    o[1] = make_uint4(ed[4], ed[5], ed[6], ed[7]);
    o[2] = make_uint4(__float_as_uint(nrm), 0u, 0u, 0u);
}

static int fused_mlp_launch(const pnr_mlp_desc* desc, const void* packed, const float* rays, const float* z, int64_t n_rays,
                            int n_samples, void* workspace, void* stream, MlpArgs& a)
{
    int rc = pnr_mlp_validate(desc);
    if (rc != PNR_OK) return rc;
    PNR_REQUIRE(desc->precision == PNR_PREC_BF16, "pnr_mlp_forward_composite: bf16 only");
    PNR_REQUIRE(desc->plan != 4, "pnr_mlp_forward_composite: a plan-4 (field) image is for pnr_mlp_query only");
    PNR_REQUIRE(n_rays >= 1 && n_samples >= 32 && n_samples <= 256 && (n_samples & 31) == 0,
                "pnr_mlp_forward_composite: n_samples=%d must be a multiple of 32 in [32,256]", n_samples);
    PNR_REQUIRE(desc->n_sem + desc->n_inst <= 128, "pnr_mlp_forward_composite: n_sem + n_inst <= 128");
    PNR_REQUIRE(packed && rays && z && workspace, "pnr_mlp_forward_composite: null pointer");
    PNR_REQUIRE(n_rays * (int64_t)n_samples < ((int64_t)1 << 31) - 4096, "pnr_mlp_forward_composite: R*N exceeds 2^31");
    PNR_REQUIRE((((uintptr_t)rays | (uintptr_t)packed | (uintptr_t)workspace) & 15) == 0,
                "pnr_mlp_forward_composite: rays / packed / workspace must be 16-byte aligned");
    PnrPlan plan;
    pnr_build_plan(*desc, plan);
    mlp_args_fill(a, desc, plan, packed);
    a.rays = rays; a.z = z; a.S = (int)(n_rays * n_samples); a.N = n_samples;
    pnr_set_div_magic(n_samples, a.n_magic, a.n_shift);
    a.rec_floats = record_floats(*desc);
    a.rec = (float*)workspace;
    const int64_t tiles = ((int64_t)a.S + 255) / 256 * 8;
    a.ps = (float4*)(a.rec + tiles * a.rec_floats);
    hipStream_t st = (hipStream_t)stream;
    const bool softmax = (desc->flags & PNR_MLP_SOFTMAX) && desc->n_sem + desc->n_inst > 0;
    if (desc->plan == 3)
        return desc->W == 256 ? launch_mlp_pp<256, false, true, 0, true>(a, st) : launch_mlp_pp<128, false, true, 0, true>(a, st);
    if (desc->plan == 2) {
        PnrTTArgs t;
        memset(&t, 0, sizeof(t));
        t.image = a.data; t.rays = rays; t.z = z; t.S = a.S; t.N = a.N; t.n_magic = a.n_magic; t.n_shift = a.n_shift;
        t.rec = a.rec; t.rec_floats = a.rec_floats; t.ps = a.ps; t.n_sem = a.n_sem; t.n_inst = a.n_inst; t.clk = a.clk;
        PNR_REQUIRE(n_rays < ((int64_t)1 << 24), "pnr_mlp_forward_composite: the two-tile kernel addresses 2^24 rays per launch");
        uint32_t* aux = (uint32_t*)(((uintptr_t)((uint8_t*)a.ps + (int64_t)a.S * 16 + 256) + PNR_RAY_AUX_BYTES - 1)
                                    & ~(uintptr_t)(PNR_RAY_AUX_BYTES - 1));
        k_ray_aux<<<dim3((unsigned)((2 * n_rays + 255) / 256)), dim3(256), 0, st>>>(rays, n_rays, aux);
        t.aux = aux;
        t.n_wg = (desc->flags >> 16) & 0x1FF;
        const bool trace = (desc->flags & 0xFF00) == PNR_MLP_TRACE;
        return pnr_mlp_tt_launch(t, (desc->n_sem + 31) / 32, (desc->n_inst + 31) / 32, a.head_depth, a.head_tap, softmax, st, trace,
                                 trace ? ((desc->flags >> 4) & 7) : 0);
    }
    if (desc->plan == 1) {
        const int nbs = (desc->n_sem + 31) / 32, nbi = (desc->n_inst + 31) / 32;
        switch (4 * nbs + nbi + (softmax ? 16 : 0)) {
        case 4: return launch_mlp_pp<256, false, true, 4>(a, st);
        case 5: return launch_mlp_pp<256, false, true, 5>(a, st);
        case 8: return launch_mlp_pp<256, false, true, 8>(a, st);
        case 9: return launch_mlp_pp<256, false, true, 9>(a, st);
        case 20: return launch_mlp_pp<256, false, true, 20>(a, st);
        case 21: return launch_mlp_pp<256, false, true, 21>(a, st);
        case 24: return launch_mlp_pp<256, false, true, 24>(a, st);
        case 25: return launch_mlp_pp<256, false, true, 25>(a, st);
        default: PNR_REQUIRE(false, "pnr_mlp_forward_composite: no plan-1 kernel for %d + %d logit blocks", nbs, nbi);
        }
    }
    PNR_REQUIRE(!softmax, "pnr_mlp_forward_composite: softmax compositing needs the plan-1 image (pnr_mlp_fused_plan >= 1, desc.plan = 1)");
    return desc->W == 256 ? launch_mlp_pp<256, false, true>(a, st) : launch_mlp_pp<128, false, true>(a, st);
}

PNR_EXPORT int pnr_mlp_forward_tiles(const pnr_mlp_desc* desc, const void* packed, const float* rays, const float* z, int64_t n_rays,
                                     int n_samples, void* workspace, void* stream)
{
    PNR_REQUIRE(n_rays >= 0, "pnr_mlp_forward_tiles: bad size");
    if (n_rays == 0) return PNR_OK;
    MlpArgs a;
    return fused_mlp_launch(desc, packed, rays, z, n_rays, n_samples, workspace, stream, a);
}

PNR_EXPORT int pnr_composite_combine(const pnr_mlp_desc* desc, const void* workspace, const float* z, int64_t n_rays, int n_samples,
                                     const int32_t* label_sem, const int32_t* label_inst, int white_bkgd, float* rgb, float* depth,
                                     float* acc, float* weights, float* sem, float* inst, float* fix_sem, float* fix_inst, void* stream)
{
    int rc = pnr_mlp_validate(desc);
    if (rc != PNR_OK) return rc;
    PNR_REQUIRE(n_rays >= 0 && n_samples >= 32 && n_samples <= 256 && (n_samples & 31) == 0, "pnr_composite_combine: bad size");
    if (n_rays == 0) return PNR_OK;
    PNR_REQUIRE(workspace && z, "pnr_composite_combine: null pointer");
    PNR_REQUIRE(desc->plan != 4, "pnr_composite_combine: a plan-4 (field) image has no compositing workspace");
    PNR_REQUIRE((!fix_sem || label_sem) && (!fix_inst || label_inst), "pnr_composite_combine: fix_* outputs need their labels");
    PNR_REQUIRE(desc->plan != 3 || (!rgb && !sem && !inst), "pnr_composite_combine: a plan-3 (sigma-only) workspace has no rgb, semantic "
                "or instance maps: pass null for them");
    const int rf = record_floats(*desc);
    const int64_t tiles = (n_rays * n_samples + 255) / 256 * 8;
    const float* rec = (const float*)workspace;
    return pnr_composite_combine_launch(rec, rf, desc->plan != 3, (const float4*)(rec + tiles * rf), z, fix_sem ? label_sem : nullptr,
                                        fix_inst ? label_inst : nullptr, n_rays, n_samples, desc->n_sem, desc->n_inst, white_bkgd,
                                        rgb, depth, acc, weights, sem, inst, fix_sem, fix_inst, (hipStream_t)stream);
}

PNR_EXPORT int pnr_mlp_forward_composite(const pnr_mlp_desc* desc, const void* packed, const float* rays, const float* z,
                                         int64_t n_rays, int n_samples, const int32_t* label_sem, const int32_t* label_inst,
                                         int white_bkgd, float* rgb, float* depth, float* acc, float* weights, float* sem,
                                         float* inst, float* fix_sem, float* fix_inst, void* workspace, void* stream)
{
    PNR_REQUIRE(n_rays >= 0, "pnr_mlp_forward_composite: bad size");
    if (n_rays == 0) return PNR_OK;
    PNR_REQUIRE((!fix_sem || label_sem) && (!fix_inst || label_inst), "pnr_mlp_forward_composite: fix_* outputs need their labels");
    PNR_REQUIRE(!desc || desc->plan != 3 || (!rgb && !sem && !inst), "pnr_mlp_forward_composite: a plan-3 (sigma-only) image has no "
                "rgb, semantic or instance maps: pass null for them");
    MlpArgs a;
    int rc = fused_mlp_launch(desc, packed, rays, z, n_rays, n_samples, workspace, stream, a);
    if (rc != PNR_OK) return rc;
    return pnr_composite_combine_launch(a.rec, a.rec_floats, desc->plan != 3, a.ps, z, fix_sem ? label_sem : nullptr, fix_inst ? label_inst : nullptr,
                                        n_rays, n_samples, desc->n_sem, desc->n_inst, white_bkgd, rgb, depth, acc, weights, sem, inst,
                                        fix_sem, fix_inst, (hipStream_t)stream);
}

PNR_EXPORT int pnr_mlp_forward_train(const pnr_mlp_desc* desc, const void* packed, const float* rays, const float* z,
                                     int64_t n_rays, int n_samples, float* raw, int64_t raw_stride_s,
                                     int64_t raw_stride_c, void* acts, void* stream)
{
    PNR_REQUIRE(acts || n_rays == 0, "pnr_mlp_forward_train: acts is null");
    return mlp_forward_impl(desc, packed, rays, z, n_rays, n_samples, raw, raw_stride_s, raw_stride_c, acts, stream);
}

PNR_EXPORT int pnr_mlp_train_layout(const pnr_mlp_desc* desc, int64_t n_samples, int64_t* acts_off_host,
                                    int64_t* dys_off_host)
{
    int rc = pnr_mlp_validate(desc);
    if (rc != PNR_OK) return rc;
    PNR_REQUIRE(acts_off_host && dys_off_host && n_samples >= 0, "pnr_mlp_train_layout: bad arguments");
    int64_t a[24], d[24];
    pnr_train_layout(*desc, n_samples, a, d);
    memcpy(acts_off_host, a, sizeof(int64_t) * (size_t)(desc->D + 7));
    memcpy(dys_off_host, d, sizeof(int64_t) * (size_t)(desc->D + 8));
    return PNR_OK;
}

struct FieldArgs {
    MlpArgs m;
    const float* pts;
    float* sigma;
    int32_t* sem_label; int32_t* inst_label; int32_t* panoptic;
    const int32_t* is_thing;
    float* sem_logits; float* inst_logits; int64_t lstride;
    int run_sem, run_inst;
};

template <class CTX, int NA, class EPI>
__device__ __forceinline__ void pp_field_out(CTX& c, u32x4 (&A)[CTX::P], const uint32_t (&in)[NA], int n_out, EPI&& epi)
{
    using CH = PPChunk<1, NA, 0>;
    const uint32_t dummy[1] = {0};
    const int nfb = (n_out + 31) >> 5;
#pragma unroll 1
    for (int fb = 0; fb < nfb; ++fb) {
        f32x16 acc[1];
        CH::prologue(c.frag_addr(), c.bias_addr(), A, acc);
        CH::mma(c.frag_addr(), A, in, dummy, acc, [&](auto... k) { if constexpr (sizeof...(k) == 0) { c.stamp(6); c.barrier(); c.stamp(2); } else c.stamp(k...); });
        c.m_done();
        c.refill_begin();
        c.refill_one();
        epi(fb, acc[0]);
        c.refill_rest();
        c.advance();
    }
}

struct FieldBest { float v; int i; };
__device__ __forceinline__ void field_best_merge(FieldBest& b, int hi)
{
    const auto pv = __builtin_amdgcn_permlane32_swap(__float_as_uint(b.v), __float_as_uint(b.v), false, false);
    const auto pi = __builtin_amdgcn_permlane32_swap((uint32_t)b.i, (uint32_t)b.i, false, false);
    const float ov = __uint_as_float(hi ? pv[0] : pv[1]);
    const int oi = (int)(hi ? pi[0] : pi[1]);
    if (ov > b.v || (ov == b.v && oi < b.i)) { b.v = ov; b.i = oi; }
    if (b.i == 0x7fffffff) b.i = 0;
}

template <int W, bool HEADS>
__global__ __launch_bounds__(512, 2) void k_mlp_pp_field(const FieldArgs fa)
{
    constexpr int WAVES = 8;
    using CTX = CtxPP<WAVES>;
    extern __shared__ __attribute__((aligned(16))) char smem[];
    constexpr int NFB = W / 32, HFB = W / 64;
    constexpr int HR = NFB * 8, GR = HFB * 8, GXR = 16;
    const MlpArgs& a = fa.m;
    CTX c = pp_ctx<WAVES>(a, smem);
    unsigned long long clk_c0, clk_r0;
    pp_begin(c, clk_c0, clk_r0);
    const int n = c.lane & 31;

    uint32_t dummy[1] = {0};
    u32x4 A[CTX::P];
// ... 122 lines not shown
```

panopticnerf_amd/csrc/pnr_mlp_pack.cpp:

```cpp
#include <math.h>
#include <string.h>

#include <vector>

#include "pnr_common.h"
#include "pnr_mlp_layout.h"
#include "pnr_mlp_plan.h"
#include "pnr_mlp_tt.h"

int pnr_mlp_validate(const pnr_mlp_desc* d)
{
    PNR_REQUIRE(d, "pnr_mlp: null desc");
    PNR_REQUIRE(d->W == 256 || d->W == 128, "pnr_mlp: W=%d unsupported (128 or 256)", d->W);
    PNR_REQUIRE(d->D >= 2 && d->D <= 16, "pnr_mlp: D=%d outside [2,16]", d->D);
    PNR_REQUIRE(d->skip >= -1 && d->skip < d->D - 1, "pnr_mlp: skip=%d must be -1 or < D-1", d->skip);
    PNR_REQUIRE(d->xyz_L >= 0 && d->xyz_L <= 10, "pnr_mlp: xyz_L=%d outside [0,10]", d->xyz_L);
    PNR_REQUIRE(d->dir_L >= 0 && d->dir_L <= 4, "pnr_mlp: dir_L=%d outside [0,4]", d->dir_L);
    PNR_REQUIRE(d->n_sem >= 0 && d->n_sem <= 256 && d->n_inst >= 0 && d->n_inst <= 256,
                "pnr_mlp: n_sem/n_inst outside [0,256]");
    PNR_REQUIRE((d->n_sem == 0 && d->n_inst == 0) || d->head_W == d->W / 2,
                "pnr_mlp: head_W=%d must equal W/2=%d", d->head_W, d->W / 2);
    PNR_REQUIRE(d->precision == PNR_PREC_BF16 || d->precision == PNR_PREC_FP32, "pnr_mlp: bad precision %d",
                d->precision);
    PNR_REQUIRE(d->head_tap == 0 || d->head_tap == 1, "pnr_mlp: head_tap=%d must be 0 (trunk output) or 1 (feature)", d->head_tap);
    PNR_REQUIRE(d->head_depth >= 0 && d->head_depth <= 2, "pnr_mlp: head_depth=%d must be 1 or 2", d->head_depth);
    PNR_REQUIRE(d->schedule >= 0 && d->schedule <= 2, "pnr_mlp: schedule=%d must be 0 (default), 1 (lock-step) or 2 (ping-pong)", d->schedule);
    PNR_REQUIRE(d->plan == 0 || (d->plan == 1 && pnr_plan1_supported(*d)) || (d->plan == 2 && pnr_plan2_supported(*d)) ||
                (d->plan == 3 && pnr_plan3_supported(*d)) || (d->plan == 4 && pnr_plan4_supported(*d)),
                "pnr_mlp: plan=%d is not available for this geometry (ask pnr_mlp_fused_plan; plans 3 and 4: bf16 only)", d->plan);
    const uint32_t trace = (uint32_t)d->flags & 0xFF00u;
    PNR_REQUIRE(((uint32_t)d->flags & ~(uint32_t)(PNR_MLP_SOFTMAX | 0xFF70u | PNR_MLP_WG_CAP(0x1FF))) == 0 && (trace == 0 || trace == PNR_MLP_TRACE) &&
                (trace != 0 || ((uint32_t)d->flags & 0x70u) == 0),
                "pnr_mlp: unknown bits in flags=0x%x (zero-initialise pnr_mlp_desc; PNR_MLP_* are the defined bits)", (unsigned)d->flags);
    PNR_REQUIRE(((uint32_t)d->clk_probe[0] & 15u) == 0, "pnr_mlp: clk_probe=0x%08x%08x is not a 16-byte aligned device address "
                "(zero-initialise pnr_mlp_desc; clk_probe is a diagnostics field, 0 = off)", (unsigned)d->clk_probe[1], (unsigned)d->clk_probe[0]);
    PNR_REQUIRE(trace == 0 || (d->clk_probe[0] | d->clk_probe[1]) != 0, "pnr_mlp: PNR_MLP_TRACE needs clk_probe");
    return PNR_OK;
}

PNR_EXPORT int pnr_mlp_fused_plan(const pnr_mlp_desc* desc)
{
    if (!desc) return 0;
    pnr_mlp_desc d = *desc;
    d.plan = 0;
    if (pnr_mlp_validate(&d) != PNR_OK) return 0;
    return pnr_plan2_supported(d) ? 2 : pnr_plan1_supported(d) ? 1 : 0;
}

PNR_EXPORT int pnr_mlp_query_supported(const pnr_mlp_desc* desc)
{
    if (!desc) return 0;
    pnr_mlp_desc d = *desc;
    d.plan = 0;
    if (pnr_mlp_validate(&d) != PNR_OK) return 0;
    return pnr_plan4_supported(d);
}

static int bwd_validate(const pnr_mlp_desc* d)
{
    int rc = pnr_mlp_validate(d);
    if (rc != PNR_OK) return rc;
    PNR_REQUIRE(d->plan == 0, "pnr_mlp backward: plan must be 0");
    PNR_REQUIRE(d->precision == PNR_PREC_BF16, "pnr_mlp backward: bf16 only");
    PNR_REQUIRE(d->n_sem <= PNR_BWD_OUT_SLOTS && d->n_inst <= PNR_BWD_OUT_SLOTS,
                "pnr_mlp backward: n_sem / n_inst must be <= %d", PNR_BWD_OUT_SLOTS);
    return PNR_OK;
}

static int check_params(const pnr_mlp_desc* desc, const pnr_mlp_params_host* p, bool bias)
{
    PNR_REQUIRE(p, "pnr_mlp_pack: null params");
    if (desc->plan == 3) {
        PNR_REQUIRE(p->pts_w && p->alpha_w && (!bias || (p->pts_b && p->alpha_b)), "pnr_mlp_pack: missing trunk or alpha_linear parameter");
        return PNR_OK;
    }
    if (desc->plan == 4) {
        const bool feat = desc->head_tap == 1 && (desc->n_sem || desc->n_inst);
        PNR_REQUIRE(p->pts_w && p->alpha_w && (!bias || (p->pts_b && p->alpha_b)), "pnr_mlp_pack: missing trunk or alpha_linear parameter");
        PNR_REQUIRE(!feat || (p->feature_w && (!bias || p->feature_b)), "pnr_mlp_pack: missing feature_linear parameter");
    } else {
    PNR_REQUIRE(p->pts_w && p->alpha_w && p->feature_w && p->views_w && p->rgb_w, "pnr_mlp_pack: missing trunk parameter");
    if (bias) PNR_REQUIRE(p->pts_b && p->alpha_b && p->feature_b && p->views_b && p->rgb_b, "pnr_mlp_pack: missing trunk bias");
    }
    const bool deep = pnr_head_depth(*desc) == 2;
    if (desc->n_sem) PNR_REQUIRE((!deep || p->sem0_w) && p->sem1_w && (!bias || ((!deep || p->sem0_b) && p->sem1_b)), "pnr_mlp_pack: missing semantic head");
    if (desc->n_inst) PNR_REQUIRE((!deep || p->inst0_w) && p->inst1_w && (!bias || ((!deep || p->inst0_b) && p->inst1_b)), "pnr_mlp_pack: missing instance head");
    return PNR_OK;
}

struct Image {
    pnr_pack_header hdr;
    std::vector<pnr_chunk_entry> table;
    std::vector<PnrFragDesc> frags;
    size_t table_off, data_off, total_bytes;
};

static PnrFragDesc zero_desc()
{
    PnrFragDesc f;
    memset(&f, 0, sizeof(f));
    return f;
}

static void fill_header(Image& im, const pnr_mlp_desc& d, int version, size_t n_chunks, int max_frags, size_t table_off,
                        size_t data_off, size_t total)
{
    memset(&im.hdr, 0, sizeof(im.hdr));
    im.hdr.magic = PNR_PACK_MAGIC;
    im.hdr.version = (uint32_t)version;
    im.hdr.n_chunks = (uint32_t)n_chunks;
    im.hdr.max_chunk_frags = (uint32_t)max_frags;
    im.hdr.table_off = (uint32_t)table_off;
    im.hdr.data_off = (uint32_t)data_off;
    im.hdr.total_bytes = total;
// ... 271 lines not shown
```

panopticnerf_amd/csrc/pnr_mlp_tt.cpp:

```cpp
#include <mutex>
#include <string>

#include "pnr_common.h"
#include "pnr_mlp_tt.h"

static const unsigned char k_co[] = {
#include "pnr_mlp_tt_co.inc"
};

namespace {
struct DevTable {
    hipModule_t mod = nullptr;
    hipFunction_t fn[8][4][2] = {};
    hipFunction_t fn_trace[8] = {};
    bool tried = false, ok = false;
};
DevTable g_tab[64];
std::mutex g_mu;
}

static int tt_table(DevTable*& out, int capturing = 0)
{
    int dev = 0;
    PNR_HIP(hipGetDevice(&dev));
    PNR_REQUIRE(dev >= 0 && dev < 64, "pnr_mlp_tt: device index %d out of range", dev);
    std::lock_guard<std::mutex> lk(g_mu);
    DevTable& t = g_tab[dev];
    if (!t.tried) {
        PNR_REQUIRE(!capturing, "pnr_mlp_tt: the two-tile code object is not loaded on device %d yet and the stream is capturing: make the "
                    "first plan-2 call (or pnr_mlp_pack_device / pnr_mlp_packed_bytes with plan = 2) outside the capture", dev);
        t.tried = true;
        hipError_t e = hipModuleLoadData(&t.mod, k_co);
        const bool loaded = e == hipSuccess;
        static const int geo[6][2] = {{1, 1}, {2, 1}, {0, 0}, {1, 0}, {2, 0}, {3, 0}};
        for (int k = 0; k < 6 && e == hipSuccess; ++k) {
            for (int v = 0; v < (geo[k][0] ? 8 : 1) && e == hipSuccess; ++v) {
                char tag[16], nm[64];
                snprintf(tag, sizeof(tag), "%s%s%s", (v & 4) ? "f" : "", (v & 1) ? "d1" : "", (v & 2) ? "sm" : "");
                snprintf(nm, sizeof(nm), "k_mlp_tt_%s%ss%di%d", tag, tag[0] ? "_" : "", geo[k][0], geo[k][1]);
                e = hipModuleGetFunction(&t.fn[v][geo[k][0]][geo[k][1]], t.mod, nm);
            }
        }
        for (int a = 0; a < 8 && e == hipSuccess; ++a) {
            char nm[64];
            if (a) snprintf(nm, sizeof(nm), "k_mlp_tt_s2i1_trace_a%d", a); else snprintf(nm, sizeof(nm), "k_mlp_tt_s2i1_trace");
            if (hipModuleGetFunction(&t.fn_trace[a], t.mod, nm) != hipSuccess) { t.fn_trace[a] = nullptr; (void)hipGetLastError(); }
        }
        if (e != hipSuccess) {
            pnr_set_error("pnr_mlp_tt: loading the two-tile code object failed: %s (the first call on a device must not be inside a "
                          "stream capture)", hipGetErrorString(e));
            if (loaded) (void)hipModuleUnload(t.mod);
            t = DevTable();
            (void)hipGetLastError();
            return PNR_EHIP;
        }
        t.ok = true;
    }
    PNR_REQUIRE(t.ok, "pnr_mlp_tt: the two-tile code object is not loaded");
    out = &t;
    return PNR_OK;
}

int pnr_mlp_tt_prepare(void)
{
    DevTable* t = nullptr;
    return tt_table(t);
}

void pnr_mlp_tt_prepare_quiet(void)
{
    int n = 0;
    if (hipGetDeviceCount(&n) != hipSuccess || n <= 0) { (void)hipGetLastError(); return; }
    const std::string keep = pnr_last_error();
    DevTable* t = nullptr;
    if (tt_table(t) != PNR_OK) pnr_set_error("%s", keep.c_str());
}

int pnr_mlp_tt_launch(const PnrTTArgs& a, int nbs, int nbi, int head_depth, int head_tap, bool softmax, hipStream_t stream, bool trace, int trace_abl)
{
    PNR_REQUIRE(nbs >= 0 && nbs <= 3 && nbi >= 0 && nbi <= (nbs == 1 || nbs == 2 ? 1 : 0), "pnr_mlp_forward_composite: no two-tile kernel for %d + %d logit blocks", nbs, nbi);
    PNR_REQUIRE(a.S >= 1 && a.S < (1 << 28), "pnr_mlp_forward_composite: the two-tile kernel takes R*N < 2^28 samples per launch (got %d): "
                "render in chunks", a.S);
    DevTable* t = nullptr;
    hipStreamCaptureStatus cs = hipStreamCaptureStatusNone;
    PNR_HIP(hipStreamIsCapturing(stream, &cs));
    int rc = tt_table(t, cs != hipStreamCaptureStatusNone);
    if (rc != PNR_OK) return rc;
    hipFunction_t fn = t->fn[!nbs ? 0 : (head_tap ? 4 : 0) + (softmax ? 2 : 0) + (head_depth == 1 ? 1 : 0)][nbs][nbi];
    PNR_REQUIRE(fn, "pnr_mlp_tt: no kernel for %d + %d logit blocks at head_depth %d", nbs, nbi, head_depth);
    if (trace) {
        PNR_REQUIRE(head_depth != 1 && !softmax && !head_tap, "pnr_mlp_tt: the trace build exists for head_depth 2, head_tap 0, logits compositing");
        PNR_REQUIRE(nbs == 2 && nbi == 1 && a.clk, "pnr_mlp_tt: the trace build exists for 2 + 1 logit blocks and needs the clock buffer");
        fn = t->fn_trace[trace_abl & 7];
        PNR_REQUIRE(fn, "pnr_mlp_tt: PNR_MLP_TRACE%s%d is not in this library: the trace kernels are diagnostics builds "
                    "(make EXTRA_TT=trace, ablations EXTRA_TT=abl)", trace_abl & 7 ? " ablation " : " ", trace_abl & 7);
    }
    PnrTTArgs ka = a;
    const int cus = pnr_cu_count();
    ka.n_groups = (a.S + 255) / 256;
    const int cap = (a.n_wg > 0 && a.n_wg < cus) ? a.n_wg : cus;
    ka.n_wg = ka.n_groups < cap ? ka.n_groups : cap;
    size_t size = sizeof(ka);
    void* extra[] = {HIP_LAUNCH_PARAM_BUFFER_POINTER, &ka, HIP_LAUNCH_PARAM_BUFFER_SIZE, &size, HIP_LAUNCH_PARAM_END};
    PNR_HIP(hipModuleLaunchKernel(fn, (unsigned)ka.n_wg, 1, 1, 256, 1, 1, 0, stream, nullptr, extra));
    return PNR_OK;
}
```

panopticnerf_amd/csrc/pnr_mlp_tt.h:

```cpp
#pragma once
#include <hip/hip_runtime.h>
#include <stdint.h>

struct PnrTTArgs {
    const void* image;
    const float* rays;
    const float* z;
    int32_t S, N;
    uint32_t n_magic;
    int32_t n_shift;
    int32_t n_groups, n_wg;
    float* rec;
    int32_t rec_floats, pad0;
    void* ps;
    int32_t n_sem, n_inst;
    unsigned long long* clk;
    const void* aux;
    uint64_t reserved;
};
static_assert(sizeof(PnrTTArgs) == 104, "k_mlp_tt reads its arguments at fixed offsets");

int pnr_mlp_tt_prepare(void);
void pnr_mlp_tt_prepare_quiet(void);
int pnr_mlp_tt_launch(const PnrTTArgs& a, int nbs, int nbi, int head_depth, int head_tap, bool softmax, hipStream_t stream, bool trace = false,
                      int trace_abl = 0);
```

panopticnerf_amd/ops.py:

```python
import ctypes
import functools
import math
import os

import torch

from . import _lib
from . import camera as _camera
from ._lib import MlpDesc, MlpParamsHost


def _stream():
    return ctypes.c_void_p(torch.cuda.current_stream().cuda_stream)


def _chk(t, name, dtype=torch.float32):
    if t is None:
        return None
    if not t.is_cuda:
        raise RuntimeError(f"{name}: expected a GPU tensor (the HIP path has no CPU fallback)")
    if t.dtype != dtype:
        raise TypeError(f"{name}: expected {dtype}, got {t.dtype}")
    if not t.is_contiguous():
        raise ValueError(f"{name}: tensor must be contiguous")
# ... 1359 lines not shown
        raw = out if out is not None else alloc_raw(ch, S, z.device)
        ss, sc = 1, _chk_raw(raw, ch, S)
    else:
        raw = out if out is not None else torch.empty((R, N, ch), device=z.device, dtype=torch.float32)
        ss, sc = ch, 1
        _count("mlp_forward", "out", _chk(raw, "raw"), S * ch, "(R, N, ch)")
    _on("mlp_forward", z.device, "z", out=raw)
    _lib.check(_lib.load().pnr_mlp_forward(ctypes.byref(desc), _p(packed), _p(rays), _p(z), R, N, _p(raw), ss, sc,
                                           _stream()), "pnr_mlp_forward")
    return raw


@_on_device
def composite(raw, z, rays, n_sem=0, n_inst=0, channel_major=True, noise=None, label_sem=None, label_inst=None,
              sem_mode=0, white_bkgd=False, want_weights=True, out=None):
    noise, draw = _draw_or(noise, "noise")
    R, N = _level("composite", rays, z)
    ch = 4 + n_sem + n_inst
    if channel_major:
        ss, sc = 1, _chk_raw(raw, ch, R * N)
    else:
        _count("composite", "raw", _chk(raw, "raw"), R * N * ch, "(R, N, ch)")
        ss, sc = ch, 1
    dev = z.device
    _count("composite", "noise", noise, R * N, "one per sample")
    label_sem, label_inst = _labels("composite", label_sem, label_inst, R * N, dev)
    _on("composite", dev, "z", raw=raw, noise=noise, call=draw.call if draw else None)
    out = _maps(out, R, N, n_sem, n_inst, label_sem, label_inst, want_weights, dev)
    g = out.get
    fn, nz, what = _twin("pnr_composite", noise, draw)
    _lib.check(fn(_p(raw), ss, sc, _p(z), _p(rays), nz, _p(label_sem), _p(label_inst), R, N, n_sem, n_inst, int(sem_mode),
                  int(bool(white_bkgd)), _p(out["rgb"]), _p(out["depth"]), _p(out["acc"]), _p(g("weights")), _p(g("semantic")),
                  _p(g("instance")), _p(g("fix_semantic")), _p(g("fix_instance")), _stream()), what)
    return out


def _maps(out, R, N, n_sem, n_inst, label_sem, label_inst, want_weights, dev, drop=()):
    f32 = dict(device=dev, dtype=torch.float32)
    shapes = {"rgb": (R, 3), "depth": (R,), "acc": (R,)}
    if want_weights:
        shapes["weights"] = (R, N)
    if n_sem:
        shapes["semantic"] = (R, n_sem)
        if label_sem is not None:
            shapes["fix_semantic"] = (R, n_sem)
    if n_inst:
        shapes["instance"] = (R, n_inst)
        if label_inst is not None:
            shapes["fix_instance"] = (R, n_inst)
    for k in drop:
        shapes.pop(k, None)
    res = {}
    for k, shp in shapes.items():
        t = out.get(k) if out else None
        if t is None:
            t = torch.empty(shp, **f32)
        elif tuple(t.shape) != shp or t.dtype != torch.float32 or t.device != dev or not t.is_contiguous():
            raise ValueError("out[%r] must be a contiguous fp32 tensor of shape %s on %s" % (k, shp, dev))
        res[k] = t
    return res


def fused_supported(desc, n_samples, sem_mode=0, noise=None):
    ok = (desc.precision == _lib.PREC_BF16 and int(sem_mode) in (0, 1) and noise is None and n_samples % 32 == 0
          and 32 <= n_samples <= 256 and desc.n_sem + desc.n_inst <= 128)
    if ok and int(sem_mode) == 1 and desc.n_sem + desc.n_inst > 0:
        ok = int(_lib.load().pnr_mlp_fused_plan(ctypes.byref(desc_for_mode(desc, 1)))) >= 1
    return ok


def desc_for_mode(desc, sem_mode):
    want = _lib.MLP_SOFTMAX if int(sem_mode) == 1 else 0
    if (desc.flags & _lib.MLP_SOFTMAX) == want:
        return desc
    return _desc_with(desc, flags=(desc.flags & ~_lib.MLP_SOFTMAX) | want)


def fused_image(sem_mode=0):
    return "softmax" if int(sem_mode) == 1 else True


@_on_device
def mlp_forward_composite(desc, packed, rays, z, label_sem=None, label_inst=None, white_bkgd=False, want_weights=True, out=None,
                          sem_mode=0, wg_cap=0):
    image = desc
    desc = desc_for_mode(desc, sem_mode)
    if wg_cap:
        desc = _desc_with(desc, flags=(desc.flags & 0xFFFF) | ((int(wg_cap) & 0x1FF) << 16))
    return _fused_level("mlp_forward_composite", desc, image, packed, rays, z, label_sem, label_inst, white_bkgd, want_weights, out)


def _fused_level(what, desc, image, packed, rays, z, label_sem, label_inst, white_bkgd, want_weights, out, drop=()):
    R, N = _level(what, rays, z, image, packed)
    dev = z.device
    label_sem, label_inst = _labels(what, label_sem, label_inst, R * N, dev)
    lib = _lib.load()
    nbytes = lib.pnr_mlp_forward_composite_workspace_bytes(ctypes.byref(desc), R, N, int(bool(want_weights)))
    if nbytes < 0:
        raise RuntimeError("pnr_mlp_forward_composite: unsupported geometry (n_samples=%d must be a multiple of 32)" % N)
    ws = torch.empty(int(nbytes), device=dev, dtype=torch.uint8)
    out = _maps(out, R, N, desc.n_sem, desc.n_inst, label_sem, label_inst, want_weights, dev, drop=drop)
    g = out.get
    _lib.check(lib.pnr_mlp_forward_composite(ctypes.byref(desc), _p(packed), _p(rays), _p(z), R, N, _p(label_sem), _p(label_inst),
                                             int(bool(white_bkgd)), _p(g("rgb")), _p(out["depth"]), _p(out["acc"]),
                                             _p(g("weights")), _p(g("semantic")), _p(g("instance")), _p(g("fix_semantic")),
                                             _p(g("fix_instance")), _p(ws), _stream()), "pnr_mlp_forward_composite")
    return out


WEIGHTS_ONLY_DROPS = ("rgb", "semantic", "instance")


def sigma_pass_supported(desc, n_samples, noise=None):
    if not (desc.precision == _lib.PREC_BF16 and noise is None and n_samples % 32 == 0 and 32 <= n_samples <= 256
            and desc.n_sem + desc.n_inst <= 128):
        return False
    return int(_lib.load().pnr_mlp_packed_bytes(ctypes.byref(_desc_with(desc, plan=3)))) > 0


@_on_device
def mlp_forward_weights(desc, packed, rays, z, label_sem=None, label_inst=None, out=None):
    if desc.plan != 3:
        raise ValueError("mlp_forward_weights: needs the plan-3 image (net.packed(level, device, fused='sigma')), not plan %d" % desc.plan)
    return _fused_level("mlp_forward_weights", desc, desc, packed, rays, z, label_sem, label_inst, False, True, out, WEIGHTS_ONLY_DROPS)


QUERY_WANTS = ("sigma", "labels", "panoptic", "logits")


def field_query_supported(desc):
    return bool(_lib.load().pnr_mlp_query_supported(ctypes.byref(desc)))


def query_keys(desc, want):
    want = (want,) if isinstance(want, str) else tuple(want)
    bad = [w for w in want if w not in QUERY_WANTS]
    if bad:
        raise ValueError("query: unknown output %r in want (known: %s)" % (bad[0], ", ".join(QUERY_WANTS)))
    keys = []
    if "sigma" in want:
        keys.append("sigma")
    if "labels" in want:
        keys += (["sem_label"] if desc.n_sem else []) + (["inst_label"] if desc.n_inst else [])
    if "panoptic" in want and desc.n_sem:
        keys.append("panoptic")
    if "logits" in want:
        keys += (["sem_logits"] if desc.n_sem else []) + (["inst_logits"] if desc.n_inst else [])
    if not keys:
        raise ValueError("query: want=%r asks for nothing this network has (n_sem=%d, n_inst=%d)" % (want, desc.n_sem, desc.n_inst))
    return keys


@_on_device
def mlp_query(desc, packed, points, want=("sigma", "labels"), is_thing=None, out=None):
    if desc.plan != 4:
        raise ValueError("mlp_query: needs the plan-4 image (net.packed(level, device, fused='field')), not plan %d" % desc.plan)
    keys = query_keys(desc, want)
    points = _chk(points, "points")
    is_thing = _chk(is_thing, "is_thing", torch.int32)
    if points.dim() != 2 or points.shape[1] != 3:
        raise ValueError("mlp_query: points must be (P, 3), got %s" % (tuple(points.shape),))
    if is_thing is not None and (not desc.n_sem or is_thing.numel() != desc.n_sem):
        raise ValueError("mlp_query: is_thing must hold n_sem=%d entries of a network with a semantic head" % desc.n_sem)
    P, dev = points.shape[0], points.device
    _packed("mlp_query", desc, packed)
    _on("mlp_query", dev, "points", packed=packed, is_thing=is_thing)
    out = dict(out) if out else {}
    res, stride = {}, P
    for k in keys:
# ... 242 lines not shown
```

panopticnerf_amd/renderer.py:

```python
import collections
import os

import torch

from . import ops


Prims = collections.namedtuple("Prims", "planes offsets")


def _get(cfg, name, default):
    return getattr(cfg, name, default) if cfg is not None else default


CHUNK_QUANTUM = 1024
CHUNK_TAIL = 8


def chunk_plan(n_rays, chunk_size):
    n_rays, chunk_size = int(n_rays), max(1, int(chunk_size))
    if n_rays <= 0:
        return []
    n = -(-n_rays // chunk_size)
    if n > 1 and n_rays - (n - 1) * chunk_size <= chunk_size // CHUNK_TAIL:
        n -= 1
    size = -(-n_rays // n)
    if n > 1 and chunk_size >= CHUNK_QUANTUM * CHUNK_TAIL:
        size = -(-size // CHUNK_QUANTUM) * CHUNK_QUANTUM
    out, s = [], 0
    while s < n_rays:
        e = min(n_rays, s + size)
        out.append((s, e))
        s = e
    return out


def _keyed(res, z, lv):
    return {**{f"{k}_{lv}": v for k, v in res.items()}, f"z_vals_{lv}": z}


def _level_out(out, lv):
    return {k[:-2]: v for k, v in out.items() if k.endswith(f"_{lv}") and k != f"z_vals_{lv}"}


def _fill_rows(rows, o):
    for k, v in o.items():
        if v.data_ptr() != rows[k].data_ptr():
            rows[k].copy_(v)


def _unflatten(maps, lead):
    return {k: v if v.dim() == 0 else v.reshape(*lead, *v.shape[1:]) for k, v in maps.items()}


def merge_chunks(outs):
    if len(outs) == 1:
        return outs[0]
    ret = {}
    for k in outs[0]:
        vs = [o[k] for o in outs]
        head, lv = k.rsplit("_", 1)
        if vs[0].dim() > 0:
            ret[k] = torch.cat(vs, 0)
        elif head.endswith("_n"):
            ret[k] = torch.stack(vs).sum()
        else:
            n = torch.stack([o[f"{head}_n_{lv}"] for o in outs])
            ret[k] = (torch.stack(vs) * n).sum() / n.sum().clamp(min=1.0)
    return ret


class Renderer:
    def __init__(self, net, cfg=None):
        self.net = net
        self.cfg = cfg
        self.N_samples = _get(cfg, "N_samples", 64)
        self.N_importance = _get(cfg, "N_importance", _get(cfg, "cascade_samples", 0))
        self.chunk_size = _get(cfg, "chunk_size", 65536)
        self.perturb = _get(cfg, "perturb", 0.0)
        self.raw_noise_std = _get(cfg, "raw_noise_std", 0.0)
        self.white_bkgd = _get(cfg, "white_bkgd", False)
        self.lindisp = _get(cfg, "lindisp", False)
        self.max_hits = _get(cfg, "max_hits", 8)
        self.sem_mode = {"none": 0, "logits": 0, "softmax": 1}[_get(cfg, "semantic_activation", "none")]
        self.keep_weights = _get(cfg, "keep_weights", True)
        self.fuse = bool(_get(cfg, "fuse_composite", os.environ.get("PNR_FUSE", "1") != "0"))
        self.strict_hits = bool(_get(cfg, "strict_hits", False))
        self.coarse_outputs = _get(cfg, "coarse_outputs", "all")
        if self.coarse_outputs not in ("all", "weights"):
            raise ValueError("cfg.coarse_outputs must be 'all' or 'weights', not %r" % (self.coarse_outputs,))
        if self.coarse_outputs == "weights" and self.N_importance <= 0:
            raise ValueError("cfg.coarse_outputs = 'weights' needs a fine level (N_importance > 0): without one the coarse maps are "
                             "the render's output")
        self.bbox_sampling = _get(cfg, "bbox_sampling", "none")
        if self.bbox_sampling not in ("none", "hull"):
            raise ValueError("cfg.bbox_sampling must be 'none' or 'hull', not %r" % (self.bbox_sampling,))
        self._overflow = None
        self.rng = _get(cfg, "rng", "torch")
        if self.rng not in ("torch", "device"):
            raise ValueError("cfg.rng must be 'torch' or 'device', not %r" % (self.rng,))
        self.rng_state = None
        if self.rng == "device":
            seed = _get(cfg, "rng_seed", None)
            seed = torch.initial_seed() if seed is None else int(seed)
            seed = (seed + 2 ** 63) % 2 ** 64 - 2 ** 63
            p0 = next(iter(net.parameters()), None)
            self.rng_state = torch.tensor([seed, 0], dtype=torch.int64, device=p0.device if p0 is not None else "cpu")
        self.frame_outputs = bool(_get(cfg, "frame_outputs", os.environ.get("PNR_FRAME_OUT", "1") != "0"))
        self.overlap_levels = bool(_get(cfg, "overlap_levels", os.environ.get("PNR_OVERLAP", "1") != "0"))
        self._side_streams = {}
        if self.N_importance > 0 and getattr(net, "nerf_1", None) is None and not getattr(net, "share_coarse_fine", False):
            raise ValueError("make_renderer: cfg asks for a fine pass (N_importance / cascade_samples = %d) but the network "
                             "was built without a fine NeRF -- build it with make_network(cfg) from the SAME cfg, or set "
                             "cfg.share_coarse_fine = True to evaluate one NeRF at both levels on purpose" % self.N_importance)

    def _preamble(self, rays, box, box_ids, t_rand, z_out):
        hits = lab0 = None
        hull = self.bbox_sampling == "hull"
        prims = isinstance(box, Prims)
        if box is not None and not prims and self.max_hits <= ops.RAY_SETUP_MAX_HITS:
            hits, z, ls0, li0 = ops.ray_setup(rays, box, box_ids, self.N_samples, self.max_hits, self.lindisp, t_rand, hull, out=z_out)
            lab0 = (ls0, li0)
        else:
            if prims:
                hits = ops.convex_hits(rays, box.planes, box.offsets, self.max_hits)
            elif box is not None:
                hits = ops.bbox_hits(rays, box, self.max_hits)
            rays_s = ops.restrict_rays(rays, hits[0], hits[2]) if (hits is not None and hull) else rays
            z = ops.stratified(rays_s, self.N_samples, self.lindisp, t_rand, out=z_out)
        return hits, z, lab0

    def _labels(self, z, hits, box_ids, lab=None):
        if lab is not None:
            return lab
        return ops.sample_labels(z, hits[0], hits[1], hits[2], box_ids) if hits is not None else (None, None)

    def _noise(self, lv, z, train, rng):
        if not (self.raw_noise_std > 0 and train):
            return None
        if rng is not None:
            return ops.Draw(rng[0], 3 + lv, rng[1], self.raw_noise_std)
        return torch.randn(z.shape, device=z.device) * self.raw_noise_std

    def _need_weights(self, lv):
        return self.keep_weights or (lv == 0 and self.N_importance > 0)

    def _level(self, lv, rays, z, labels, noise, out, grad, wg_cap=0):
        net, dev = self.net, rays.device
        ls, li = labels
        n0 = net.nerf(0)
        if grad:
            from . import train as _train
            return _train.level_train(self, lv, rays, z, ls, li, noise)
        weights_only = lv == 0 and self.coarse_outputs == "weights"
        need_w = self._need_weights(lv)
        d = net.nerf(lv).desc(net.precision)
        if weights_only and self.fuse and ops.sigma_pass_supported(d, z.shape[1], noise):
            desc, img = net.packed(0, dev, fused="sigma")
            return ops.mlp_forward_weights(desc, img, rays, z, ls, li, out=out)
        if not weights_only and self.fuse and ops.fused_supported(d, z.shape[1], self.sem_mode, noise):
            desc, img = net.packed(lv, dev, fused=ops.fused_image(self.sem_mode))
            return ops.mlp_forward_composite(desc, img, rays, z, ls, li, self.white_bkgd, need_w, out=out, sem_mode=self.sem_mode,
                                             wg_cap=wg_cap)
        desc, img = net.packed(lv, dev)
        raw = ops.mlp_forward(desc, img, rays, z, channel_major=True)
        res = ops.composite(raw, z, rays, n0.n_sem, n0.n_inst, True, noise, ls, li, self.sem_mode, self.white_bkgd, need_w, out=out)
        return {k: v for k, v in res.items() if k not in ops.WEIGHTS_ONLY_DROPS} if weights_only else res

    def _resample(self, z, weights, hits, box_ids, u, z_out):
        w0 = weights.detach().contiguous()
        if hits is not None:
            z_fine, ls1, li1 = ops.sample_pdf_labels(z, w0, self.N_importance, hits, box_ids, u, out=z_out)
            return z_fine, (ls1, li1)
        z_fine, _, _ = ops.sample_pdf(z, w0, self.N_importance, u, want_samples=False, out=z_out)
        return z_fine, None

    def render_rays(self, rays, box=None, box_ids=None, t_rand=None, u=None, train=False, grad=False, out=None, rng=None):
        Nc, Nf = self.N_samples, self.N_importance
        dev = rays.device
        out = out if (out and not grad) else {}
        draw = self.perturb > 0 and train
        if t_rand is None and draw:
            t_rand = ops.Draw(rng[0], 1, rng[1]) if rng is not None else torch.rand((rays.shape[0], Nc), device=dev)
        hits, z, lab0 = self._preamble(rays, box, box_ids, t_rand, out.get("z_vals_0"))
        if hits is not None and self.strict_hits:
            over = torch.stack([(hits[2] > self.max_hits).sum(), hits[2].max()])
            self._overflow = over if self._overflow is None else torch.stack([self._overflow[0] + over[0],
                                                                              torch.maximum(self._overflow[1], over[1])])
        lab0 = self._labels(z, hits, box_ids, lab0)
        o0 = self._level(0, rays, z, lab0, self._noise(0, z, train, rng), _level_out(out, 0), grad)
        ret = _keyed(o0, z, 0)
        if Nf > 0:
            if u is None and draw:
                u = ops.Draw(rng[0], 2, rng[1]) if rng is not None else torch.rand((rays.shape[0], Nf), device=dev)
            z_fine, lab1 = self._resample(z, o0["weights"], hits, box_ids, u, out.get("z_vals_1"))
            lab1 = self._labels(z_fine, hits, box_ids, lab1)
            o1 = self._level(1, rays, z_fine, lab1, self._noise(1, z_fine, train, rng), _level_out(out, 1), grad)
            ret.update(_keyed(o1, z_fine, 1))
        return ret

    def _output_maps(self, R, has_box, dev, grad=False):
        n0 = self.net.nerf(0)
        lab = True if has_box else None
        Nc, Nf = self.N_samples, self.N_importance
        ret = {}
        for lv, N in ((0, Nc), (1, Nc + Nf)) if Nf > 0 else ((0, Nc),):
            drop = ops.WEIGHTS_ONLY_DROPS if (lv == 0 and not grad and self.coarse_outputs == "weights") else ()
            m = ops._maps(None, R, N, n0.n_sem, n0.n_inst, lab, lab, self._need_weights(lv), dev, drop=drop)
            ret.update(_keyed(m, torch.empty((R, N), device=dev, dtype=torch.float32), lv))
        return ret

    def _empty_outputs(self, lead, has_box, dev, grad=False):
        return _unflatten(self._output_maps(0, has_box, dev, grad), lead)

    def _overlap_caps(self, dev, plan, grad, train, has_box, t_rand, u):
        if (not self.overlap_levels or grad or train or len(plan) < 2 or not self.fuse or not self.frame_outputs or self.N_importance <= 0
                or self.strict_hits or t_rand is not None or u is not None or self.raw_noise_std > 0 and train
                or self.coarse_outputs == "weights" or torch.cuda.is_current_stream_capturing()):
            return None
        net, Nc, Nt = self.net, self.N_samples, self.N_samples + self.N_importance
        for lv, N in ((0, Nc), (1, Nt)):
            d = net.nerf(lv).desc(net.precision)
            if not ops.fused_supported(d, N, self.sem_mode, None) or net.packed(lv, dev, fused=ops.fused_image(self.sem_mode))[0].plan != 2:
                return None
        cus = torch.cuda.get_device_properties(dev).multi_processor_count
        cap_c = int(round(cus * Nc / float(Nc + Nt) / 8.0)) * 8
        cap_f = cus - cap_c
        if cus % 8 or cap_c < 8 or cap_f < 8 or abs((Nc / float(cap_c)) / (Nt / float(cap_f)) - 1.0) > 0.05:
            return None
        return cap_c, cap_f

    def _render_overlapped(self, rays, box, box_ids, plan, caps, lead):
        dev = rays.device
        cap_c, cap_f = caps
        last = len(plan) - 1
        frame = self._output_maps(rays.shape[0], box is not None, dev)
        main = torch.cuda.current_stream(dev)
        if dev not in self._side_streams:
            self._side_streams[dev] = (torch.cuda.Stream(dev), torch.cuda.Stream(dev))
        side = self._side_streams[dev]
        start = torch.cuda.Event()
        start.record(main)
        for st in side:
            st.wait_event(start)
        prev_pdf = None
        pre = {}
# ... 127 lines not shown
```

Before: 1177.

## Fuse ray compositing into the two-tile MLP kernel with a finishing variant

Adds a 'fin' variant of the generated two-tile MLP assembly kernel that composites each ray in the epilogue: transmittance weights, depth/acc/rgb accumulation via LDS carries across steps, sigmoid colour, label histograms and fixed-label maps, plus wave reductions and direct stores of the final maps. Work is reassigned so each wave walks whole rays in 64-sample steps rather than arbitrary sample tiles. It is enabled by default through PNR_FINISH. The aim is to drop the separate composite pass and the round trip of per-sample records through global memory. In exchange it adds epilogue instructions, LDS traffic and serial per-ray dependencies that could lengthen the MLP kernel.

```diff
diff --git a/include/pnr.h b/include/pnr.h
--- a/include/pnr.h
+++ b/include/pnr.h
@@ -41,6 +41,7 @@
 
 #define PNR_MLP_SOFTMAX 1
 #define PNR_MLP_WG_CAP(n) (((n) & 0x1FF) << 16)
+#define PNR_MLP_NO_FINISH 4
 #define PNR_MLP_TRACE 0x7A00
 
 typedef struct pnr_mlp_params_host {
diff --git a/panopticnerf_amd/_lib.py b/panopticnerf_amd/_lib.py
--- a/panopticnerf_amd/_lib.py
+++ b/panopticnerf_amd/_lib.py
@@ -9,7 +9,7 @@
 c_int = ctypes.c_int
 
 PREC_BF16, PREC_FP32 = 0, 1
-MLP_SOFTMAX, MLP_TRACE = 1, 0x7A00
+MLP_SOFTMAX, MLP_NO_FINISH, MLP_TRACE = 1, 4, 0x7A00
 CAMERA_PINHOLE, CAMERA_FISHEYE, CAMERA_EQUIRECT = 0, 1, 3
 TAG_PIXEL, TAG_FRAME = 16, 17
 SAMPLE_POOLED, SAMPLE_FRAME = 0, 1
diff --git a/panopticnerf_amd/csrc/asm/gen_mlp_tt.py b/panopticnerf_amd/csrc/asm/gen_mlp_tt.py
--- a/panopticnerf_amd/csrc/asm/gen_mlp_tt.py
+++ b/panopticnerf_amd/csrc/asm/gen_mlp_tt.py
@@ -36,6 +36,15 @@
 S_K = 100
 S_Q = 19
 S_GRP2 = 29
+S_LABS, S_LABI, S_ORGB, S_ODEP, S_OACC, S_OW, S_OSEM, S_OINST, S_OFS, S_OFI = 32, 80, 84, 86, 88, 90, 92, 94, 76, 78
+S_Q0, S_WHITE = 3, S_REC_I
+S_RAYP = S_REC_T
+HIST_BASE = LW_BASE + 1024
+CARRY_BASE = HIST_BASE + 4 * 512
+S_TA, S_TB, S_TNEXT = 16, 17, 18
+S_LASTV = 72
+S_STEPS, S_J, S_J2 = 20, 21, 71
+FIN_KERNARG_BYTES = 192
 
 
 def f32(x):
@@ -88,7 +97,9 @@
 
 
 class Gen:
-    def __init__(self, nbs, nbi, name, trace=False, abl=0, depth=2, softmax=False, tap=0):
+    def __init__(self, nbs, nbi, name, trace=False, abl=0, depth=2, softmax=False, tap=0, finish=False):
+        self.finish = finish
+        assert not finish or (depth == 2 and not softmax and not tap and not trace)
         self.depth = depth
         self.tap = tap
         self.softmax = softmax
@@ -484,11 +495,19 @@
         e = self.e
         vi = V_IN + 8 * t
         s_, sl, ray, a64 = V_PTMP, V_PTMP + 1, V_PTMP + 2, V_PTMP + 4
-        e("s_lshl_b32 s%d, s%d, 3" % (S_T0, grp_sreg))
-        e("s_lshl_b32 s%d, s%d, 1" % (S_T1, S_WAVE))
-        e("s_add_u32 s%d, s%d, s%d" % (S_T0, S_T0, S_T1))
-        e("s_add_u32 s%d, s%d, %d" % (S_T0, S_T0, t))
-        e("s_lshl_b32 s%d, s%d, 5" % (S_T0, S_T0))
+        if self.finish:
+            e("s_lshl_b32 s%d, s%d, 2" % (S_T0, grp_sreg))
+            e("s_add_u32 s%d, s%d, s%d" % (S_T0, S_T0, S_WAVE))
+            e("s_mul_i32 s%d, s%d, s%d" % (S_T0, S_T0, S_N))
+            e("s_lshl_b32 s%d, s%d, 6" % (S_T1, S_J2))
+            e("s_add_u32 s%d, s%d, s%d" % (S_T0, S_T0, S_T1))
+            e("s_add_u32 s%d, s%d, %d" % (S_T0, S_T0, 32 * t))
+        else:
+            e("s_lshl_b32 s%d, s%d, 3" % (S_T0, grp_sreg))
+            e("s_lshl_b32 s%d, s%d, 1" % (S_T1, S_WAVE))
+            e("s_add_u32 s%d, s%d, s%d" % (S_T0, S_T0, S_T1))
+            e("s_add_u32 s%d, s%d, %d" % (S_T0, S_T0, t))
+            e("s_lshl_b32 s%d, s%d, 5" % (S_T0, S_T0))
         e("v_and_b32 v%d, 31, v%d" % (s_, V_TID))
         e("v_or_b32 v%d, s%d, v%d" % (s_, S_T0, s_))
         e("v_cmp_gt_i32 s[%d:%d], s%d, v%d" % (S_NVALID + 2 * t, S_NVALID + 2 * t + 1, S_S, s_))
@@ -628,6 +647,8 @@
             e("v_mov_b32 v%d, 1.0" % n)
             e("s_nop 1")
             e("v_readlane_b32 s%d, v%d, 31" % (S_Q, f))
+            if self.finish and t == 0:
+                e("v_readlane_b32 s%d, v%d, 31" % (S_Q0, f))
             e("v_mov_b32_dpp v%d, v%d wave_shr:1 row_mask:0xf bank_mask:0xf" % (n, f))
             e("v_cndmask_b32 v%d, v%d, 1.0, s[%d:%d]" % (n, n, S_N0, S_N0 + 1))
             e("v_mul_f32 v%d, v%d, v%d" % (V_LW + t, al, n))
@@ -669,7 +690,248 @@
             e("v_mov_b32 v%d, 0" % d)
             self.vm_op("global_store_dword v%d, v%d, s[%d:%d]" % (d, x, S_REC_T + 2 * t, S_REC_T + 2 * t + 1))
             e("s_mov_b64 exec, -1")
-        self.q(28, stores)
+        if not self.finish:
+            self.q(28, stores)
+
+    def fin_exec(self, ptr, lanes=None, valid=S_VALID):
+        e = self.e
+        src = valid
+        if lanes is not None:
+            e("s_and_b64 s[%d:%d], s[%d:%d], %s" % (S_SAVE, S_SAVE + 1, valid, valid + 1, lanes))
+            src = S_SAVE
+        e("s_cmp_lg_u64 s[%d:%d], 0" % (ptr, ptr + 1))
+        e("s_cselect_b64 exec, s[%d:%d], 0" % (src, src + 1))
+
+    def fin_ray(self):
+        self.e("s_lshl_b32 s%d, s%d, 2" % (S_T0, S_GRP))
+        self.e("s_add_u32 s%d, s%d, s%d" % (S_T0, S_T0, S_WAVE))
+
+    def fin_first_mask(self):
+        self.e("s_cmp_eq_u32 s%d, 0" % S_J)
+        self.e("s_cselect_b64 s[%d:%d], -1, 0" % (S_RAYP, S_RAYP + 1))
+
+    def fin_hist_base(self):
+        self.e("s_lshl_b32 s%d, s%d, 9" % (S_T1, S_WAVE))
+        self.e("s_add_u32 s%d, s%d, 0x%x" % (S_T1, S_T1, HIST_BASE))
+
+    def fin_expf(self, y, x, d, n):
+        e = self.e
+        self.lit(S_K, 0x3fb8aa3b)
+        e("v_mul_f32 v%d, 0x3fb8aa3b, v%d" % (y, x))
+        e("v_fma_f32 v%d, v%d, s%d, -v%d" % (d, x, S_K, y))
+        e("v_rndne_f32 v%d, v%d" % (n, y))
+        e("v_fmac_f32 v%d, 0x32a5705f, v%d" % (d, x))
+        e("v_sub_f32 v%d, v%d, v%d" % (y, y, n))
+        e("v_add_f32 v%d, v%d, v%d" % (y, y, d))
+        e("v_exp_f32 v%d, v%d" % (y, y))
+        e("v_cvt_i32_f32 v%d, v%d" % (n, n))
+        e("s_nop 0")
+        e("v_ldexp_f32 v%d, v%d, v%d" % (y, y, n))
+        self.lit(S_K, 0xc2ce8ed0)
+        e("v_cmp_ngt_f32 s[%d:%d], s%d, v%d" % (S_T0, S_T0 + 1, S_K, x))
+        e("v_cndmask_b32 v%d, 0, v%d, s[%d:%d]" % (y, y, S_T0, S_T0 + 1))
+        self.lit(S_K, 0x42b17218)
+        e("v_cmp_nlt_f32 s[%d:%d], s%d, v%d" % (S_T0, S_T0 + 1, S_K, x))
+        e("v_mov_b32 v%d, 0x7f800000" % n)
+        e("v_cndmask_b32 v%d, v%d, v%d, s[%d:%d]" % (y, n, y, S_T0, S_T0 + 1))
+
+    def finish_rays(self, accs, release):
+        e = self.e
+        T = list(range(V_TMP, V_TMP + 16))
+        P = list(range(V_PTMP, V_PTMP + 8))
+        W, Z, CR, CG, CB, ADR, LS, LI, R0, ONE, X, D, Y, NN, HL, CL = T[:16]
+        tags = {}
+
+        def gather():
+            src = ((W, V_LW, V_LW + 1), (Z, V_ZZ, V_ZZ + 1), (CR, accs[0], accs[1]), (CG, accs[0] + 1, accs[1] + 1),
+                   (CB, accs[0] + 2, accs[1] + 2))
+            for k, (d_, s0, s1) in enumerate(src):
+                e("v_mov_b32 v%d, v%d" % (d_, s0))
+                e("v_mov_b32 v%d, v%d" % (P[k], s1))
+            with self.atomic():
+                e("s_nop 1")
+                for k, (d_, s0, s1) in enumerate(src):
+                    e("v_permlane32_swap_b32 v%d, v%d" % (d_, P[k]))
+                e("s_nop 1")
+        self.q(20, gather)
+        self.q(0, release)
+
+        def labels():
+            with self.atomic():
+                e("s_add_u32 s%d, s%d, 1" % (S_T0, S_J))
+                e("s_cmp_eq_u32 s%d, s%d" % (S_T0, S_STEPS))
+                e("s_cselect_b64 s[%d:%d], s[%d:%d], 0" % (S_LASTV, S_LASTV + 1, S_VALID, S_VALID + 1))
+                self.fin_ray()
+                e("s_mul_i32 s%d, s%d, s%d" % (S_T0, S_T0, S_N))
+                e("s_lshl_b32 s%d, s%d, 6" % (S_T1, S_J))
+                e("s_add_u32 s%d, s%d, s%d" % (S_T0, S_T0, S_T1))
+                e("v_and_b32 v%d, 63, v%d" % (ADR, V_TID))
+                e("v_or_b32 v%d, s%d, v%d" % (ADR, S_T0, ADR))
+                e("v_lshlrev_b32 v%d, 2, v%d" % (ADR, ADR))
+            e("v_mov_b32 v%d, -1" % LS)
+            e("v_mov_b32 v%d, -1" % LI)
+            for reg, ptr in ((LS, S_LABS), (LI, S_LABI)):
+                with self.atomic():
+                    self.fin_exec(ptr)
+                    tags[reg] = self.vm_op("global_load_dword v%d, v%d, s[%d:%d]" % (reg, ADR, ptr, ptr + 1), certain=False)
+                    e("s_mov_b64 exec, -1")
+            with self.atomic():
+                self.fin_hist_base()
+                e("v_and_b32 v%d, 63, v%d" % (HL, V_TID))
+                e("v_lshl_add_u32 v%d, v%d, 2, s%d" % (HL, HL, S_T1))
+                e("v_mov_b32 v%d, 0" % P[6])
+                e("s_cmp_eq_u32 s%d, 0" % S_J)
+                e("s_cselect_b64 exec, -1, 0")
+                self.lds_read("ds_write_b32 v%d, v%d" % (HL, P[6]))
+                self.lds_read("ds_write_b32 v%d, v%d offset:256" % (HL, P[6]))
+                e("s_mov_b64 exec, -1")
+            with self.atomic():
+                e("s_lshl_b32 s%d, s%d, 11" % (S_T1, S_WAVE))
+                e("s_add_u32 s%d, s%d, 0x%x" % (S_T1, S_T1, CARRY_BASE))
+                e("v_and_b32 v%d, 63, v%d" % (CL, V_TID))
+                e("v_lshl_add_u32 v%d, v%d, 2, s%d" % (CL, CL, S_T1))
+            self.lds_read("ds_read_b32 v%d, v%d" % (R0, CL))
+            tags[R0] = self.lds_read("ds_read_b32 v%d, v%d offset:256" % (ONE, CL))
+        self.q(24, labels)
+
+        def weights():
+            with self.atomic():
+                e("s_cmp_eq_u32 s%d, 0" % S_J)
+                e("s_cselect_b32 s%d, 1.0, s%d" % (S_TA, S_TNEXT))
+            e("v_mov_b32 v%d, s%d" % (P[0], S_TA))
+            e("v_mul_f32 v%d, s%d, v%d" % (P[1], S_Q0, P[0]))
+            e("v_mul_f32 v%d, s%d, v%d" % (P[2], S_Q, P[1]))
+            e("v_readfirstlane_b32 s%d, v%d" % (S_TB, P[1]))
+            e("v_readfirstlane_b32 s%d, v%d" % (S_TNEXT, P[2]))
+            e("v_cndmask_b32 v%d, v%d, v%d, s[%d:%d]" % (P[0], P[1], P[0], S_LO32, S_LO32 + 1))
+            e("v_mul_f32 v%d, v%d, v%d" % (W, P[0], W))
+            with self.atomic():
+                self.fin_exec(S_OW)
+                self.vm_op("global_store_dword v%d, v%d, s[%d:%d]" % (ADR, W, S_OW, S_OW + 1), certain=False)
+                e("s_mov_b64 exec, -1")
+            self.wait_lgkm(tags[R0])
+            with self.atomic():
+                self.fin_first_mask()
+                e("v_cndmask_b32 v%d, v%d, 0, s[%d:%d]" % (R0, R0, S_RAYP, S_RAYP + 1))
+                e("v_cndmask_b32 v%d, v%d, 0, s[%d:%d]" % (ONE, ONE, S_RAYP, S_RAYP + 1))
+            e("v_add_f32 v%d, v%d, v%d" % (R0, R0, W))
+            e("v_fma_f32 v%d, v%d, v%d, v%d" % (Z, W, Z, ONE))
+            self.lds_read("ds_write_b32 v%d, v%d" % (CL, R0))
+            self.lds_read("ds_write_b32 v%d, v%d offset:256" % (CL, Z))
+        self.q(10, weights)
+
+        def sigmoid(c, k):
+            prev = self.lds_read("ds_read_b32 v%d, v%d offset:%d" % (P[4], CL, 256 * k))
+            e("v_xor_b32 v%d, 0x80000000, v%d" % (X, c))
+            self.fin_expf(Y, X, D, NN)
+            e("v_add_f32 v%d, 1.0, v%d" % (Y, Y))
+            e("v_mov_b32 v%d, 1.0" % ONE)
+            self.div(X, ONE, Y, [D, NN, P[1], P[2], P[3]])
+            self.wait_lgkm(prev)
+            with self.atomic():
+                self.fin_first_mask()
+                e("v_cndmask_b32 v%d, v%d, 0, s[%d:%d]" % (P[4], P[4], S_RAYP, S_RAYP + 1))
+            e("v_fma_f32 v%d, v%d, v%d, v%d" % (c, W, X, P[4]))
+            self.lds_read("ds_write_b32 v%d, v%d offset:%d" % (CL, c, 256 * k))
+        for k, c in enumerate((CR, CG, CB)):
+            self.q(36, (lambda c=c, k=k: sigmoid(c, 2 + k)))
+
+        def hist():
+            self.wait_vm(tags[LS])
+            self.wait_vm(tags[LI])
+            e("v_mul_f32 v%d, 0x4e800000, v%d" % (P[2], W))
+            e("v_add_f32 v%d, 0.5, v%d" % (P[2], P[2]))
+            e("v_cvt_u32_f32 v%d, v%d" % (P[2], P[2]))
+            for lab, n_, inst in ((LS, S_NSEM, False), (LI, S_NINST, True)):
+                with self.atomic():
+                    self.fin_hist_base()
+                    e("v_cmp_gt_u32 s[%d:%d], s%d, v%d" % (S_SAVE, S_SAVE + 1, n_, lab))
+                    if inst:
+                        e("v_add_u32 v%d, s%d, v%d" % (P[3], S_NSEM, lab))
+                        e("v_lshl_add_u32 v%d, v%d, 2, s%d" % (P[3], P[3], S_T1))
+                    else:
+                        e("v_lshl_add_u32 v%d, v%d, 2, s%d" % (P[3], lab, S_T1))
+                    e("s_and_b64 exec, s[%d:%d], s[%d:%d]" % (S_SAVE, S_SAVE + 1, S_VALID, S_VALID + 1))
+                    self.lds_read("ds_add_u32 v%d, v%d" % (P[3], P[2]))
+                    e("s_mov_b64 exec, -1")
+        self.q(20, hist)
+
+        def reduce():
+            regs = (R0, Z, CR, CG, CB)
+            e("s_nop 1")
+            for ctrl in ("quad_perm:[1,0,3,2]", "quad_perm:[2,3,0,1]", "row_half_mirror", "row_mirror"):
+                for r in regs:
+                    e("v_add_f32_dpp v%d, v%d, v%d %s row_mask:0xf bank_mask:0xf" % (r, r, r, ctrl))
+            for swap in ("v_permlane16_swap_b32", "v_permlane32_swap_b32"):
+                for k, r in enumerate(regs):
+                    e("v_mov_b32 v%d, v%d" % (P[k], r))
+                with self.atomic():
+                    e("s_nop 1")
+                    for k, r in enumerate(regs):
+                        e("%s v%d, v%d" % (swap, r, P[k]))
+                    e("s_nop 1")
+                for k, r in enumerate(regs):
+                    e("v_add_f32 v%d, v%d, v%d" % (r, r, P[k]))
+        self.q(50, reduce)
+
+        def maps():
+            with self.atomic():
+                self.fin_ray()
+                e("s_lshl_b32 s%d, s%d, 2" % (S_T1, S_T0))
+                e("v_mov_b32 v%d, s%d" % (P[0], S_T1))
+                self.fin_exec(S_OACC, "1", S_LASTV)
+                self.vm_op("global_store_dword v%d, v%d, s[%d:%d]" % (P[0], R0, S_OACC, S_OACC + 1), certain=False)
+                self.fin_exec(S_ODEP, "1", S_LASTV)
+                self.vm_op("global_store_dword v%d, v%d, s[%d:%d]" % (P[0], Z, S_ODEP, S_ODEP + 1), certain=False)
+                e("s_mov_b64 exec, -1")
+                e("v_mov_b32 v%d, v%d" % (P[1], CB))
+                e("s_mov_b64 s[%d:%d], 2" % (S_RAYP, S_RAYP + 1))
+                e("v_cndmask_b32 v%d, v%d, v%d, s[%d:%d]" % (P[1], P[1], CG, S_RAYP, S_RAYP + 1))
+                e("s_mov_b64 s[%d:%d], 1" % (S_RAYP, S_RAYP + 1))
+                e("v_cndmask_b32 v%d, v%d, v%d, s[%d:%d]" % (P[1], P[1], CR, S_RAYP, S_RAYP + 1))
+                e("v_sub_f32 v%d, 1.0, v%d" % (P[2], R0))
+                e("v_add_f32 v%d, v%d, v%d" % (P[2], P[1], P[2]))
+                e("s_cmp_lg_u32 s%d, 0" % S_WHITE)
+                e("s_cselect_b64 s[%d:%d], -1, 0" % (S_RAYP, S_RAYP + 1))
+                e("v_cndmask_b32 v%d, v%d, v%d, s[%d:%d]" % (P[1], P[1], P[2], S_RAYP, S_RAYP + 1))
+                e("s_mul_i32 s%d, s%d, 12" % (S_T1, S_T0))
+                e("v_and_b32 v%d, 63, v%d" % (P[3], V_TID))
+                e("v_lshlrev_b32 v%d, 2, v%d" % (P[3], P[3]))
+                e("v_add_u32 v%d, s%d, v%d" % (P[3], S_T1, P[3]))
+                self.fin_exec(S_ORGB, "7", S_LASTV)
+                self.vm_op("global_store_dword v%d, v%d, s[%d:%d]" % (P[3], P[1], S_ORGB, S_ORGB + 1), certain=False)
+                e("s_mov_b64 exec, -1")
+        self.q(30, maps)
+
+        def fixed():
+            h = [self.lds_read("ds_read_b32 v%d, v%d" % (P[4], HL)), self.lds_read("ds_read_b32 v%d, v%d offset:256" % (P[5], HL))]
+            self.wait_lgkm(h[1])
+            for r in (P[4], P[5]):
+                e("v_cvt_f32_u32 v%d, v%d" % (r, r))
+                e("v_mul_f32 v%d, 0x30800000, v%d" % (r, r))
+            with self.atomic():
+                self.fin_ray()
+                for k, (n_, ptr) in enumerate(((S_NSEM, S_OFS), (S_NINST, S_OFI))):
+                    e("s_mul_i32 s%d, s%d, s%d" % (S_T1, S_T0, n_))
+                    e("s_lshl_b32 s%d, s%d, 2" % (S_T1, S_T1))
+                    e("s_add_u32 s%d, s%d, s%d" % (S_RAYP + 2 * k, ptr, S_T1))
+                    e("s_addc_u32 s%d, s%d, 0" % (S_RAYP + 2 * k + 1, ptr + 1))
+                e("v_and_b32 v%d, 63, v%d" % (P[6], V_TID))
+                for hh, val in enumerate((P[4], P[5])):
+                    if hh:
+                        e("v_add_u32 v%d, 64, v%d" % (P[6], P[6]))
+                    e("v_cmp_gt_u32 s[%d:%d], s%d, v%d" % (S_SAVE, S_SAVE + 1, S_NSEM, P[6]))
+                    e("v_lshlrev_b32 v%d, 2, v%d" % (P[7], P[6]))
+                    self.fin_exec(S_OFS, "s[%d:%d]" % (S_SAVE, S_SAVE + 1), S_LASTV)
+                    self.vm_op("global_store_dword v%d, v%d, s[%d:%d]" % (P[7], val, S_RAYP, S_RAYP + 1), certain=False)
+                    e("s_mov_b64 exec, -1")
+                    e("v_subrev_u32 v%d, s%d, v%d" % (P[7], S_NSEM, P[6]))
+                    e("v_cmp_gt_u32 s[%d:%d], s%d, v%d" % (S_SAVE, S_SAVE + 1, S_NINST, P[7]))
+                    e("v_lshlrev_b32 v%d, 2, v%d" % (P[7], P[7]))
+                    self.fin_exec(S_OFI, "s[%d:%d]" % (S_SAVE, S_SAVE + 1), S_LASTV)
+                    self.vm_op("global_store_dword v%d, v%d, s[%d:%d]" % (P[7], val, S_RAYP + 2, S_RAYP + 3), certain=False)
+                    e("s_mov_b64 exec, -1")
+        self.q(40, fixed)
 
     def acc_reg(self, i):
         return V_ACC + 16 * i
@@ -933,7 +1195,10 @@
             for t in range(2):
                 self.rgbs_epilogue(t, self.acc_reg(u["accs"][(0, t)]))
             ids = list(u["accs"].values())
-            self.q(0, lambda: self.defer(lambda: self.acc_release(ids)))
+            if self.finish:
+                self.finish_rays([self.acc_reg(u["accs"][(0, t)]) for t in range(2)], lambda: self.defer(lambda: self.acc_release(ids)))
+            else:
+                self.q(0, lambda: self.defer(lambda: self.acc_release(ids)))
             self.queue_inputs_late()
             self.acc_release([self.g2_acc])
             self.g2_acc = None
@@ -1115,13 +1380,46 @@
                 base = (S_REC_I if inst else S_REC_T) + 2 * t
                 self.vm_op("global_store_dword v%d, v%d, s[%d:%d] offset:%d" % (V_LB4, oth[t][k], base, base + 1, 4 + 128 * blk))
             e("s_mov_b64 exec, -1")
+        def finish_stores():
+            for t in (0, 1):
+                for k in range(nb):
+                    self.wait_lgkm(tags[t][k])
+                    e("v_add_f32 v%d, v%d, v%d" % (oth[t][k], sums[t][k], oth[t][k]))
+            e("s_lshl_b32 s%d, s%d, 11" % (S_T1, S_WAVE))
+            e("s_add_u32 s%d, s%d, 0x%x" % (S_T1, S_T1, CARRY_BASE + 1280))
+            e("v_add_u32 v%d, s%d, v%d" % (adr, S_T1, V_LB4))
+            prev = [self.lds_read("ds_read_b32 v%d, v%d offset:%d" % (sums[1][k], adr, 128 * k)) for k in range(nb)]
+            self.fin_first_mask()
+            for k in range(nb):
+                self.wait_lgkm(prev[k])
+                e("v_cndmask_b32 v%d, v%d, 0, s[%d:%d]" % (sums[1][k], sums[1][k], S_RAYP, S_RAYP + 1))
+                e("v_fma_f32 v%d, s%d, v%d, v%d" % (sums[0][k], S_TA, oth[0][k], sums[1][k]))
+                e("v_fma_f32 v%d, s%d, v%d, v%d" % (sums[0][k], S_TB, oth[1][k], sums[0][k]))
+            e("s_mov_b64 exec, s[%d:%d]" % (S_HI0, S_HI0 + 1))
+            for k in range(nb):
+                self.lds_read("ds_write_b32 v%d, v%d offset:%d" % (adr, sums[0][k], 128 * k))
+            e("s_mov_b64 exec, -1")
+            self.fin_ray()
+            for i, (n_, ptr) in enumerate(((S_NSEM, S_OSEM), (S_NINST, S_OINST))):
+                e("s_mul_i32 s%d, s%d, s%d" % (S_T1, S_T0, n_))
+                e("s_lshl_b32 s%d, s%d, 2" % (S_T1, S_T1))
+                e("s_add_u32 s%d, s%d, s%d" % (S_RAYP + 2 * i, ptr, S_T1))
+                e("s_addc_u32 s%d, s%d, 0" % (S_RAYP + 2 * i + 1, ptr + 1))
+            for k, (u, bi, blk, inst) in enumerate(blocks):
+                self.fin_exec(S_OINST if inst else S_OSEM, "s[%d:%d]" % (S_MSK + 2 * k, S_MSK + 2 * k + 1), S_LASTV)
+                base = S_RAYP + (2 if inst else 0)
+                self.vm_op("global_store_dword v%d, v%d, s[%d:%d] offset:%d" % (V_LB4, sums[0][k], base, base + 1, 128 * blk), certain=False)
+            e("s_mov_b64 exec, -1")
         self.stamp(len(self.units) + 4)
         if self.softmax:
             self.tail_softmax(blocks, lwr_reg, tag_lwr)
         fmas((0, 1))
         self.stamp(len(self.units) + 5)
-        stores(0)
-        stores(1)
+        if self.finish:
+            finish_stores()
+        else:
+            stores(0)
+            stores(1)
         for u in self.logit_units:
             self.acc_release(list(u["accs"].values()))
         self.acc_release(self.lwr_acc)
@@ -1131,6 +1429,16 @@
     def queue_inputs_early(self):
         def which():
             with self.atomic():
+                if self.finish:
+                    self.e("s_add_u32 s%d, s%d, 1" % (S_J2, S_J))
+                    self.e("s_cmp_lt_u32 s%d, s%d" % (S_J2, S_STEPS))
+                    self.e("s_cselect_b32 s%d, 0, s%d" % (S_T0, S_NWG))
+                    self.e("s_cselect_b32 s%d, s%d, 0" % (S_J2, S_J2))
+                    self.e("s_add_u32 s%d, s%d, s%d" % (S_GRP2, S_GRP, S_T0))
+                    self.e("s_cmp_lt_i32 s%d, s%d" % (S_GRP2, S_NGRP))
+                    self.e("s_cselect_b32 s%d, s%d, s%d" % (S_GRP2, S_GRP2, S_GRP))
+                    self.e("s_cselect_b32 s%d, s%d, s%d" % (S_J2, S_J2, S_J))
+                    return
                 self.e("s_add_u32 s%d, s%d, s%d" % (S_GRP2, S_GRP, S_NWG))
                 self.e("s_cmp_lt_i32 s%d, s%d" % (S_GRP2, S_NGRP))
                 self.e("s_cselect_b32 s%d, s%d, s%d" % (S_GRP2, S_GRP2, S_GRP))
@@ -1221,12 +1529,24 @@
             self.o.append("\ts_waitcnt lgkmcnt(0)")
             self.stamp(len(self.units) + 3)
 
+    def lds_bytes(self):
+        return NSLOT * SLOT + 1024 + (4 * 512 + 4 * 2048 if self.finish else 0)
+
+    def kernarg_bytes(self):
+        return FIN_KERNARG_BYTES if self.finish else KERNARG_BYTES
+
     def kernel(self):
         e, name = self.e, self.name
         self.o += ["\t.text", "\t.globl\t%s" % name, "\t.p2align\t8", "\t.type\t%s,@function" % name, "%s:" % name]
         for dst, off, n in ((S_IMG, 0x0, 2), (S_RAYS, 0x8, 2), (S_Z, 0x10, 2), (S_S, 0x18, 2), (S_MAGIC, 0x20, 2), (S_NGRP, 0x28, 2),
                             (S_REC, 0x30, 2), (S_RECF, 0x38, 1), (S_PS, 0x40, 2), (S_NSEM, 0x48, 2), (S_CLK, 0x50, 2), (S_AUX, 0x58, 2)):
+            if self.finish and dst in (S_REC, S_RECF, S_PS):
+                continue
             e("s_load_dword%s %s, s[0:1], 0x%x" % ("x2" if n == 2 else "", sr(dst, n), off))
+        if self.finish:
+            for k, dst in enumerate((S_LABS, S_LABI, S_ORGB, S_ODEP, S_OACC, S_OW, S_OSEM, S_OINST, S_OFS, S_OFI)):
+                e("s_load_dwordx2 %s, s[0:1], 0x%x" % (sr(dst, 2), KERNARG_BYTES + 8 * k))
+            e("s_load_dword s%d, s[0:1], 0x%x" % (S_WHITE, KERNARG_BYTES + 80))
         e("v_readfirstlane_b32 s%d, v0" % S_WAVE)
         e("s_nop 4")
         e("s_lshr_b32 s%d, s%d, 6" % (S_WAVE, S_WAVE))
@@ -1270,6 +1590,10 @@
                         e("v_add_u32 v%d, %d, v%d" % (V_T0, 32 * (nblk - 1), V_T0))
                     e("v_cmp_gt_i32 s[%d:%d], s%d, v%d" % (S_VMSK + 2 * k, S_VMSK + 2 * k + 1, sreg, V_T0))
         lend, lloop, lfin = self.label(), self.label(), self.label()
+        if self.finish:
+            e("s_lshr_b32 s%d, s%d, 6" % (S_STEPS, S_N))
+            e("s_mov_b32 s%d, 0" % S_J)
+            e("s_mov_b32 s%d, 0" % S_J2)
         e("s_mov_b32 s%d, s2" % S_GRP)
         e("s_cmp_ge_i32 s%d, s%d" % (S_GRP, S_NGRP))
         e("s_cbranch_scc1 %s" % lend)
@@ -1306,9 +1630,17 @@
         self.o = keep
         self.o.append(lloop + ":")
         self.group_body()
+        if self.finish:
+            lstep = self.label()
+            e("s_add_u32 s%d, s%d, 1" % (S_J, S_J))
+            e("s_cmp_lt_u32 s%d, s%d" % (S_J, S_STEPS))
+            e("s_cbranch_scc1 %s" % lstep)
+            e("s_mov_b32 s%d, 0" % S_J)
         e("s_add_u32 s%d, s%d, s%d" % (S_GRP, S_GRP, S_NWG))
         e("s_cmp_ge_i32 s%d, s%d" % (S_GRP, S_NGRP))
         e("s_cbranch_scc1 %s" % lend)
+        if self.finish:
+            self.o.append(lstep + ":")
         self.prefetch_first_unit()
         e("s_branch %s" % lloop)
         self.o.append(lend + ":")
@@ -1362,8 +1694,8 @@
         e("s_endpgm")
         self.o += [".Lend_%s:" % name, "\t.size\t%s, .Lend_%s-%s" % (name, name, name), ""]
         self.o += ["\t.rodata", "\t.p2align\t6", "\t.amdhsa_kernel %s" % name,
-                   "\t\t.amdhsa_group_segment_fixed_size %d" % (NSLOT * SLOT + 1024),
-                   "\t\t.amdhsa_private_segment_fixed_size 0", "\t\t.amdhsa_kernarg_size %d" % KERNARG_BYTES, "\t\t.amdhsa_user_sgpr_count 2",
+                   "\t\t.amdhsa_group_segment_fixed_size %d" % self.lds_bytes(),
+                   "\t\t.amdhsa_private_segment_fixed_size 0", "\t\t.amdhsa_kernarg_size %d" % self.kernarg_bytes(), "\t\t.amdhsa_user_sgpr_count 2",
                    "\t\t.amdhsa_user_sgpr_kernarg_segment_ptr 1", "\t\t.amdhsa_system_sgpr_workgroup_id_x 1",
                    "\t\t.amdhsa_system_vgpr_workitem_id 0", "\t\t.amdhsa_next_free_vgpr 512", "\t\t.amdhsa_next_free_sgpr 102",
                    "\t\t.amdhsa_accum_offset 256", "\t\t.amdhsa_reserve_vcc 1", "\t\t.amdhsa_float_denorm_mode_32 3",
@@ -1375,12 +1707,13 @@
 KERNARG_BYTES = 104
 
 
-def metadata(names):
+def metadata(names, sizes=None):
     o = ["\t.amdgpu_metadata", "---", "amdhsa.kernels:"]
     for n in names:
-        o += ["  - .agpr_count:     256", "    .args:", "      - .offset:         0", "        .size:           %d" % KERNARG_BYTES,
-              "        .value_kind:     by_value", "    .group_segment_fixed_size: %d" % (NSLOT * SLOT + 1024),
-              "    .kernarg_segment_align: 8", "    .kernarg_segment_size: %d" % KERNARG_BYTES, "    .max_flat_workgroup_size: 256",
+        karg, lds = (sizes or {}).get(n, (KERNARG_BYTES, NSLOT * SLOT + 1024))
+        o += ["  - .agpr_count:     256", "    .args:", "      - .offset:         0", "        .size:           %d" % karg,
+              "        .value_kind:     by_value", "    .group_segment_fixed_size: %d" % lds,
+              "    .kernarg_segment_align: 8", "    .kernarg_segment_size: %d" % karg, "    .max_flat_workgroup_size: 256",
               "    .name:           %s" % n, "    .private_segment_fixed_size: 0", "    .sgpr_count:     108",
               "    .sgpr_spill_count: 0", "    .symbol:         %s.kd" % n, "    .uniform_work_group_size: 1",
               "    .uses_dynamic_stack: false", "    .vgpr_count:     512", "    .vgpr_spill_count: 0", "    .wavefront_size: 64"]
@@ -1410,6 +1743,13 @@
                     n = variant_name(tap, depth, sm, nbs, nbi)
                     names.append(n)
                     parts.append(Gen(nbs, nbi, n, depth=depth, softmax=sm, tap=tap).kernel())
+    sizes = {}
+    for nbs, nbi in ((1, 1), (2, 1), (0, 0), (1, 0), (2, 0), (3, 0)):
+        n = "k_mlp_tt_fin_s%di%d" % (nbs, nbi)
+        names.append(n)
+        g = Gen(nbs, nbi, n, finish=True)
+        parts.append(g.kernel())
+        sizes[n] = (g.kernarg_bytes(), g.lds_bytes())
     extra = sys.argv[3] if len(sys.argv) > 3 else ""
     if extra in ("trace", "abl"):
         names.append("k_mlp_tt_s2i1_trace")
@@ -1421,7 +1761,7 @@
     unit_names = ["%s %s" % (g.layers[u["layer"]]["name"], u["blocks"]) for g in [Gen(2, 1, "x")] for u in g.units]
     if len(sys.argv) > 2:
         open(sys.argv[2], "w").write("\n".join(unit_names) + "\n")
-    parts.append(metadata(names))
+    parts.append(metadata(names, sizes))
     with open(out, "w") as f:
         f.write("\n".join(parts))
 
diff --git a/panopticnerf_amd/csrc/pnr_mlp.hip b/panopticnerf_amd/csrc/pnr_mlp.hip
--- a/panopticnerf_amd/csrc/pnr_mlp.hip
+++ b/panopticnerf_amd/csrc/pnr_mlp.hip
@@ -836,7 +836,8 @@
 }
 
 static int fused_mlp_launch(const pnr_mlp_desc* desc, const void* packed, const float* rays, const float* z, int64_t n_rays,
-                            int n_samples, void* workspace, void* stream, MlpArgs& a)
+                            int n_samples, void* workspace, void* stream, MlpArgs& a, const PnrTTFinArgs* fin = nullptr,
+                            bool* finished = nullptr)
 {
     int rc = pnr_mlp_validate(desc);
     if (rc != PNR_OK) return rc;
@@ -874,6 +875,12 @@
         t.aux = aux;
         t.n_wg = (desc->flags >> 16) & 0x1FF;
         const bool trace = (desc->flags & 0xFF00) == PNR_MLP_TRACE;
+        if (fin && !trace && !(desc->flags & PNR_MLP_NO_FINISH) && pnr_mlp_tt_can_finish(n_samples, a.head_depth, a.head_tap, softmax)) {
+            PnrTTFinArgs f = *fin;
+            f.tt = t;
+            *finished = true;
+            return pnr_mlp_tt_launch_finish(f, (desc->n_sem + 31) / 32, (desc->n_inst + 31) / 32, st);
+        }
         return pnr_mlp_tt_launch(t, (desc->n_sem + 31) / 32, (desc->n_inst + 31) / 32, a.head_depth, a.head_tap, softmax, st, trace,
                                  trace ? ((desc->flags >> 4) & 7) : 0);
     }
@@ -936,8 +943,15 @@
     PNR_REQUIRE(!desc || desc->plan != 3 || (!rgb && !sem && !inst), "pnr_mlp_forward_composite: a plan-3 (sigma-only) image has no "
                 "rgb, semantic or instance maps: pass null for them");
     MlpArgs a;
-    int rc = fused_mlp_launch(desc, packed, rays, z, n_rays, n_samples, workspace, stream, a);
-    if (rc != PNR_OK) return rc;
+    PnrTTFinArgs fin;
+    memset(&fin, 0, sizeof(fin));
+    const bool want_s = fix_sem && label_sem && desc && desc->n_sem > 0, want_i = fix_inst && label_inst && desc && desc->n_inst > 0;
+    fin.lab_s = want_s ? label_sem : nullptr; fin.lab_i = want_i ? label_inst : nullptr;
+    fin.rgb = rgb; fin.depth = depth; fin.acc = acc; fin.weights = weights; fin.sem = sem; fin.inst = inst;
+    fin.fix_sem = want_s ? fix_sem : nullptr; fin.fix_inst = want_i ? fix_inst : nullptr; fin.white_bkgd = white_bkgd ? 1 : 0;
+    bool finished = false;
+    int rc = fused_mlp_launch(desc, packed, rays, z, n_rays, n_samples, workspace, stream, a, &fin, &finished);
+    if (rc != PNR_OK || finished) return rc;
     return pnr_composite_combine_launch(a.rec, a.rec_floats, desc->plan != 3, a.ps, z, fix_sem ? label_sem : nullptr, fix_inst ? label_inst : nullptr,
                                         n_rays, n_samples, desc->n_sem, desc->n_inst, white_bkgd, rgb, depth, acc, weights, sem, inst,
                                         fix_sem, fix_inst, (hipStream_t)stream);
diff --git a/panopticnerf_amd/csrc/pnr_mlp_pack.cpp b/panopticnerf_amd/csrc/pnr_mlp_pack.cpp
--- a/panopticnerf_amd/csrc/pnr_mlp_pack.cpp
+++ b/panopticnerf_amd/csrc/pnr_mlp_pack.cpp
@@ -29,7 +29,7 @@
                 (d->plan == 3 && pnr_plan3_supported(*d)) || (d->plan == 4 && pnr_plan4_supported(*d)),
                 "pnr_mlp: plan=%d is not available for this geometry (ask pnr_mlp_fused_plan; plans 3 and 4: bf16 only)", d->plan);
     const uint32_t trace = (uint32_t)d->flags & 0xFF00u;
-    PNR_REQUIRE(((uint32_t)d->flags & ~(uint32_t)(PNR_MLP_SOFTMAX | 0xFF70u | PNR_MLP_WG_CAP(0x1FF))) == 0 && (trace == 0 || trace == PNR_MLP_TRACE) &&
+    PNR_REQUIRE(((uint32_t)d->flags & ~(uint32_t)(PNR_MLP_SOFTMAX | PNR_MLP_NO_FINISH | 0xFF70u | PNR_MLP_WG_CAP(0x1FF))) == 0 && (trace == 0 || trace == PNR_MLP_TRACE) &&
                 (trace != 0 || ((uint32_t)d->flags & 0x70u) == 0),
                 "pnr_mlp: unknown bits in flags=0x%x (zero-initialise pnr_mlp_desc; PNR_MLP_* are the defined bits)", (unsigned)d->flags);
     PNR_REQUIRE(((uint32_t)d->clk_probe[0] & 15u) == 0, "pnr_mlp: clk_probe=0x%08x%08x is not a 16-byte aligned device address "
diff --git a/panopticnerf_amd/csrc/pnr_mlp_tt.cpp b/panopticnerf_amd/csrc/pnr_mlp_tt.cpp
--- a/panopticnerf_amd/csrc/pnr_mlp_tt.cpp
+++ b/panopticnerf_amd/csrc/pnr_mlp_tt.cpp
@@ -12,6 +12,7 @@
 struct DevTable {
     hipModule_t mod = nullptr;
     hipFunction_t fn[8][4][2] = {};
+    hipFunction_t fn_fin[4][2] = {};
     hipFunction_t fn_trace[8] = {};
     bool tried = false, ok = false;
 };
@@ -40,6 +41,11 @@
                 snprintf(nm, sizeof(nm), "k_mlp_tt_%s%ss%di%d", tag, tag[0] ? "_" : "", geo[k][0], geo[k][1]);
                 e = hipModuleGetFunction(&t.fn[v][geo[k][0]][geo[k][1]], t.mod, nm);
             }
+        }
+        for (int k = 0; k < 6 && e == hipSuccess; ++k) {
+            char nm[64];
+            snprintf(nm, sizeof(nm), "k_mlp_tt_fin_s%di%d", geo[k][0], geo[k][1]);
+            e = hipModuleGetFunction(&t.fn_fin[geo[k][0]][geo[k][1]], t.mod, nm);
         }
         for (int a = 0; a < 8 && e == hipSuccess; ++a) {
             char nm[64];
@@ -76,6 +82,41 @@
     if (tt_table(t) != PNR_OK) pnr_set_error("%s", keep.c_str());
 }
 
+static void tt_grid(PnrTTArgs& ka, bool super_groups = false)
+{
+    const int cus = pnr_cu_count();
+    const int want = ka.n_wg;
+    ka.n_groups = super_groups ? (ka.S / ka.N + 3) / 4 : (ka.S + 255) / 256;
+    const int cap = (want > 0 && want < cus) ? want : cus;
+    ka.n_wg = ka.n_groups < cap ? ka.n_groups : cap;
+}
+
+bool pnr_mlp_tt_can_finish(int n_samples, int head_depth, int head_tap, bool softmax)
+{
+    return n_samples >= 64 && n_samples <= 256 && n_samples % 64 == 0 && head_depth != 1 && !head_tap && !softmax;
+}
+
+int pnr_mlp_tt_launch_finish(const PnrTTFinArgs& a, int nbs, int nbi, hipStream_t stream)
+{
+    PNR_REQUIRE(nbs >= 0 && nbs <= 3 && nbi >= 0 && nbi <= (nbs == 1 || nbs == 2 ? 1 : 0), "pnr_mlp_forward_composite: no two-tile kernel for %d + %d logit blocks", nbs, nbi);
+    PNR_REQUIRE(a.tt.S >= 1 && a.tt.S < (1 << 28), "pnr_mlp_forward_composite: the two-tile kernel takes R*N < 2^28 samples per launch (got %d): "
+                "render in chunks", a.tt.S);
+    PNR_REQUIRE(a.tt.N >= 64 && a.tt.N % 64 == 0 && a.tt.S % a.tt.N == 0, "pnr_mlp_tt: the finishing kernels take whole rays of a multiple of 64 samples");
+    DevTable* t = nullptr;
+    hipStreamCaptureStatus cs = hipStreamCaptureStatusNone;
+    PNR_HIP(hipStreamIsCapturing(stream, &cs));
+    int rc = tt_table(t, cs != hipStreamCaptureStatusNone);
+    if (rc != PNR_OK) return rc;
+    hipFunction_t fn = t->fn_fin[nbs][nbi];
+    PNR_REQUIRE(fn, "pnr_mlp_tt: no finishing kernel for %d + %d logit blocks", nbs, nbi);
+    PnrTTFinArgs ka = a;
+    tt_grid(ka.tt, true);
+    size_t size = sizeof(ka);
+    void* extra[] = {HIP_LAUNCH_PARAM_BUFFER_POINTER, &ka, HIP_LAUNCH_PARAM_BUFFER_SIZE, &size, HIP_LAUNCH_PARAM_END};
+    PNR_HIP(hipModuleLaunchKernel(fn, (unsigned)ka.tt.n_wg, 1, 1, 256, 1, 1, 0, stream, nullptr, extra));
+    return PNR_OK;
+}
+
 int pnr_mlp_tt_launch(const PnrTTArgs& a, int nbs, int nbi, int head_depth, int head_tap, bool softmax, hipStream_t stream, bool trace, int trace_abl)
 {
     PNR_REQUIRE(nbs >= 0 && nbs <= 3 && nbi >= 0 && nbi <= (nbs == 1 || nbs == 2 ? 1 : 0), "pnr_mlp_forward_composite: no two-tile kernel for %d + %d logit blocks", nbs, nbi);
@@ -96,10 +137,7 @@
                     "(make EXTRA_TT=trace, ablations EXTRA_TT=abl)", trace_abl & 7 ? " ablation " : " ", trace_abl & 7);
     }
     PnrTTArgs ka = a;
-    const int cus = pnr_cu_count();
-    ka.n_groups = (a.S + 255) / 256;
-    const int cap = (a.n_wg > 0 && a.n_wg < cus) ? a.n_wg : cus;
-    ka.n_wg = ka.n_groups < cap ? ka.n_groups : cap;
+    tt_grid(ka);
     size_t size = sizeof(ka);
     void* extra[] = {HIP_LAUNCH_PARAM_BUFFER_POINTER, &ka, HIP_LAUNCH_PARAM_BUFFER_SIZE, &size, HIP_LAUNCH_PARAM_END};
     PNR_HIP(hipModuleLaunchKernel(fn, (unsigned)ka.n_wg, 1, 1, 256, 1, 1, 0, stream, nullptr, extra));
diff --git a/panopticnerf_amd/csrc/pnr_mlp_tt.h b/panopticnerf_amd/csrc/pnr_mlp_tt.h
--- a/panopticnerf_amd/csrc/pnr_mlp_tt.h
+++ b/panopticnerf_amd/csrc/pnr_mlp_tt.h
@@ -20,6 +20,17 @@
 };
 static_assert(sizeof(PnrTTArgs) == 104, "k_mlp_tt reads its arguments at fixed offsets");
 
+struct PnrTTFinArgs {
+    PnrTTArgs tt;
+    const int32_t* lab_s;
+    const int32_t* lab_i;
+    float *rgb, *depth, *acc, *weights, *sem, *inst, *fix_sem, *fix_inst;
+    int32_t white_bkgd, pad1;
+};
+static_assert(sizeof(PnrTTFinArgs) == 192, "k_mlp_tt_fin reads its arguments at fixed offsets");
+bool pnr_mlp_tt_can_finish(int n_samples, int head_depth, int head_tap, bool softmax);
+int pnr_mlp_tt_launch_finish(const PnrTTFinArgs& a, int nbs, int nbi, hipStream_t stream);
+
 int pnr_mlp_tt_prepare(void);
 void pnr_mlp_tt_prepare_quiet(void);
 int pnr_mlp_tt_launch(const PnrTTArgs& a, int nbs, int nbi, int head_depth, int head_tap, bool softmax, hipStream_t stream, bool trace = false,
diff --git a/panopticnerf_amd/ops.py b/panopticnerf_amd/ops.py
--- a/panopticnerf_amd/ops.py
+++ b/panopticnerf_amd/ops.py
@@ -1465,9 +1465,13 @@
 
 @_on_device
 def mlp_forward_composite(desc, packed, rays, z, label_sem=None, label_inst=None, white_bkgd=False, want_weights=True, out=None,
-                          sem_mode=0, wg_cap=0):
+                          sem_mode=0, wg_cap=0, finish=None):
     image = desc
     desc = desc_for_mode(desc, sem_mode)
+    if finish is None:
+        finish = os.environ.get("PNR_FINISH", "1") != "0"
+    if bool(desc.flags & _lib.MLP_NO_FINISH) == bool(finish):
+        desc = _desc_with(desc, flags=(desc.flags & ~_lib.MLP_NO_FINISH) | (0 if finish else _lib.MLP_NO_FINISH))
     if wg_cap:
         desc = _desc_with(desc, flags=(desc.flags & 0xFFFF) | ((int(wg_cap) & 0x1FF) << 16))
     return _fused_level("mlp_forward_composite", desc, image, packed, rays, z, label_sem, label_inst, white_bkgd, want_weights, out)
diff --git a/panopticnerf_amd/renderer.py b/panopticnerf_amd/renderer.py
--- a/panopticnerf_amd/renderer.py
+++ b/panopticnerf_amd/renderer.py
@@ -85,6 +85,7 @@
         self.sem_mode = {"none": 0, "logits": 0, "softmax": 1}[_get(cfg, "semantic_activation", "none")]
         self.keep_weights = _get(cfg, "keep_weights", True)
         self.fuse = bool(_get(cfg, "fuse_composite", os.environ.get("PNR_FUSE", "1") != "0"))
+        self.finish_in_mlp = bool(_get(cfg, "finish_in_mlp", os.environ.get("PNR_FINISH", "1") != "0"))
         self.strict_hits = bool(_get(cfg, "strict_hits", False))
         self.coarse_outputs = _get(cfg, "coarse_outputs", "all")
         if self.coarse_outputs not in ("all", "weights"):
@@ -161,7 +162,7 @@
         if not weights_only and self.fuse and ops.fused_supported(d, z.shape[1], self.sem_mode, noise):
             desc, img = net.packed(lv, dev, fused=ops.fused_image(self.sem_mode))
             return ops.mlp_forward_composite(desc, img, rays, z, ls, li, self.white_bkgd, need_w, out=out, sem_mode=self.sem_mode,
-                                             wg_cap=wg_cap)
+                                             wg_cap=wg_cap, finish=self.finish_in_mlp)
         desc, img = net.packed(lv, dev)
         raw = ops.mlp_forward(desc, img, rays, z, channel_major=True)
         res = ops.composite(raw, z, rays, n0.n_sem, n0.n_inst, True, noise, ls, li, self.sem_mode, self.white_bkgd, need_w, out=out)
```

Result: no change. 1178, median of 6 (+0.1%).
